# bmhopkinson/hyslam

Measured on AMD Instinct MI355X. Metric: stereo frames/sec ORB extract+match, 1920x1080 @2000 feat, higher is better.
Workload: dtype u8

## Files before the change

### hyslam_amd/csrc/hs_api.hip

```cpp
#include "hs_plan.h"
#include "hs_track.h"
#include <atomic>
#include <climits>
#include <cmath>
#include <cstdio>
#include <cstring>
#include <mutex>
#include <string>
#include <vector>

#define HS_VERSION "hyslam_amd 0.1 (gfx950)"

template <class T, bool Pinned = false> struct HsBuf {
    T* p = nullptr; size_t cap = 0;
    HsBuf() = default;
    HsBuf(const HsBuf&) = delete; HsBuf& operator=(const HsBuf&) = delete;
    HsBuf(HsBuf&& o) noexcept : p(o.p), cap(o.cap) { o.p = nullptr; o.cap = 0; }
    HsBuf& operator=(HsBuf&& o) noexcept { if (this != &o) { release(); p = o.p; cap = o.cap; o.p = nullptr; o.cap = 0; } return *this; }
    ~HsBuf() { release(); }
    void release() { if (p) (void)(Pinned ? hipHostFree(p) : hipFree(p)); p = nullptr; cap = 0; }
    hipError_t grow(size_t count)
    {
        if (count <= cap) return hipSuccess;
        release();
        const hipError_t e = Pinned ? hipHostMalloc((void**)&p, count * sizeof(T), hipHostMallocDefault) : hipMalloc((void**)&p, count * sizeof(T));
        if (e != hipSuccess) { p = nullptr; return e; }
        cap = count;
        return Pinned ? hipSuccess : hs_poison_fresh(p, count * sizeof(T));
    }
    hipError_t grow(size_t count, hipStream_t drain)
    {
        if (count <= cap) return hipSuccess;
        const hipError_t e = hipStreamSynchronize(drain);
        return e != hipSuccess ? e : grow(count);
    }
    operator T*() const { return p; }
};
template <class T> using HsPinned = HsBuf<T, true>;

struct HsFrameStaging { HsBuf<uint8_t> d_in, d_raw; };
struct HsStereoOut {
    HsBuf<float> ur, depth; HsBuf<int32_t> bd;
    hipError_t grow(size_t entries, hipStream_t drain)
    {
        if (entries <= ur.cap && entries <= depth.cap && entries <= bd.cap) return hipSuccess;
        hipError_t e = hipStreamSynchronize(drain);
        if (e == hipSuccess) e = ur.grow(entries);
        if (e == hipSuccess) e = depth.grow(entries);
        if (e == hipSuccess) e = bd.grow(entries);
        return e;
    }
};

struct hs_orb {
    hs_orb_params p;
    int device = 0;
    std::atomic<bool> owned{true};
    std::atomic<int> refs{1};
    hipStream_t stream = nullptr;
    std::string err;
    uint16_t taps[7];
    HsKnobs knobs{};
    HsFastKnobs fast_knobs{};
    uint32_t fast_epoch = 0;
    hipStream_t s_aux = nullptr; hipEvent_t ev_sfork = nullptr, ev_sjoin = nullptr;
    bool fast_taps = false;
    std::vector<float> scale, inv_scale, sigma2, inv_sigma2;
    std::vector<int> quota;
    struct Geometry {
        int w = 0, h = 0, batch_cap = 0;
        uint64_t plan_digest = 0;
        std::vector<HsLevel> lv;
        std::vector<HsLevel> lv_n;
        int last_batch = 0; HsImg0 last_img0{};
        int last_pyr_launches = 0;
        int total_cells = 0, max_wcell = 1, max_hcell = 1;
        int fast_items = 0;
        int fast_items_n = 0;
        uint64_t cand_img_stride = 0;
        int sel_img_stride = 0;
        int max_kp = 0;
        HsBuf<HsFastItem> d_fast_items, d_fast_items_n;
        HsBuf<uint32_t> d_fast_ovf;
        HsBuf<uint8_t> d_pyr;
        HsBuf<int16_t> d_tables;
        HsBuf<uint8_t> d_qt_tabs;
        HsBuf<uint16_t> d_qkeys; HsBuf<HsFastQt> d_fast_qt;
        HsBuf<uint32_t> d_qhist; HsBuf<unsigned long long> d_qbest; uint32_t qhist_stride = 0, qbest_stride = 0;
        HsBuf<uint8_t> d_qt_rects;
        bool keys_dirty = false;
        HsBuf<uint8_t> d_pyr_tabs;
        std::vector<HsPyrFuse> pyr_fuse;
        std::vector<HsPyrChain> pyr_deep;
        std::vector<HsPyrChain> pyr_chain;
        HsBuf<uint2> d_cand; HsBuf<uint32_t> d_pts_xy, d_pts_sk; HsBuf<uint16_t> d_pt_node;
        HsBuf<int32_t> d_cand_count, d_sel_count, d_cell_count;
        HsBuf<uint32_t> d_sel;
        HsBuf<uint16_t> d_sel_perm;
    } geo;
    HsBuf<HsLevel> d_lv;
    HsBuf<uint16_t> d_taps;
    bool qt_large = false;
    bool qt_small_ok = false;
    bool keep_points = false;
    HsFrameStaging in;
    HsBuf<uint8_t> d_out;
    HsStereoOut st;
    HsBuf<int32_t> d_strip_count; HsBuf<HsStripEntry> d_strip_list;
    HsBuf<hs_keypoint> d_sm_kps; HsBuf<uint8_t> d_sm_desc; HsBuf<int32_t> d_sm_n;
    HsPinned<uint8_t> h_pin;
    HsPinned<uint8_t> h_pin_out;
    int last_stereo_launches = 2;
    const hs_keypoint* pub_kps = nullptr; const uint8_t* pub_desc = nullptr; int pub_cap = 0, pub_batch = 0;
    HsBuf<uint8_t> d_scratch;
    struct IngestSlot {
        HsFrameStaging in;
        HsBuf<uint8_t> d_out;
        HsPinned<uint8_t> h_out;
        hipEvent_t ev_in = nullptr, ev_done = nullptr, ev_out = nullptr;
        int32_t ticket = 0; bool busy = false;
        int batch = 0, pairs = 0, cap = 0;
    } slot[2];
    hipStream_t s_in = nullptr, s_out = nullptr;
    int32_t next_ticket = 1;
    hs_orb* lane2 = nullptr; hipEvent_t ev_fork = nullptr, ev_join = nullptr;
    bool prof = false;
    std::vector<hipEvent_t> ev_pool; size_t ev_used = 0;
    std::vector<int> prof_stage;
};

namespace {

inline int cv_round_f(float v) { return (int)nearbyintf(v); }

void mark(hs_orb* h, int stage, hipStream_t s)
{
    if (!h->prof) return;
    if (h->ev_used == h->ev_pool.size()) { hipEvent_t e; if (hipEventCreate(&e) != hipSuccess) return; h->ev_pool.push_back(e); }
    (void)hipEventRecord(h->ev_pool[h->ev_used++], s);
    h->prof_stage.push_back(stage);
}

void free_geometry(hs_orb* h) { h->geo = hs_orb::Geometry{}; }

template <class T> void relocate(T*& p, const void* base) { p = reinterpret_cast<T*>(reinterpret_cast<uintptr_t>(base) + reinterpret_cast<uintptr_t>(p)); }
void relocate_levels(std::vector<HsLevel>& lv, const hs_orb::Geometry& g)
{
    for (size_t l = 0; l < lv.size(); l++) {
        HsLevel& V = lv[l];
        if (l > 0) { relocate(V.base, g.d_pyr.p); relocate(V.xofs, g.d_tables.p); relocate(V.ialpha, g.d_tables.p); relocate(V.yofs, g.d_tables.p); relocate(V.ibeta, g.d_tables.p); }
        if (V.qt_ytab) { relocate(V.qt_xtab, g.d_qt_tabs.p); relocate(V.qt_ytab, g.d_qt_tabs.p); }
    }
}
void relocate_pyramid(hs_orb::Geometry& g)
{
    for (std::vector<HsPyrChain>* plan : { &g.pyr_chain, &g.pyr_deep })
        for (size_t l = 0; l < plan->size(); l++) {
            HsPyrChain& C = (*plan)[l];
            if (!C.valid) continue;
            if (l > 1) relocate(C.sbase, g.d_pyr.p);
            for (int i = 0; i < C.nstage; i++) {
                HsPyrStage& S = C.st[i];
                relocate(S.base, g.d_pyr.p); relocate(S.xt, g.d_tables.p);
                relocate(S.rows, g.d_pyr_tabs.p); relocate(S.tx, g.d_pyr_tabs.p); relocate(S.ty, g.d_pyr_tabs.p);
            }
        }
    for (size_t l = 0; l < g.pyr_fuse.size(); l++) {
        HsPyrFuse& F = g.pyr_fuse[l];
        if (!F.valid) continue;
        if (l > 1) relocate(F.sbase, g.d_pyr.p);
        relocate(F.abase, g.d_pyr.p); relocate(F.bbase, g.d_pyr.p); relocate(F.xtA, g.d_tables.p); relocate(F.xtB, g.d_tables.p);
        relocate(F.rowA, g.d_pyr_tabs.p); relocate(F.rowB, g.d_pyr_tabs.p); relocate(F.xt, g.d_pyr_tabs.p); relocate(F.yt, g.d_pyr_tabs.p);
    }
}
template <class T, class V> hipError_t upload(const HsBuf<T>& d, const std::vector<V>& v)
{
    return v.empty() ? hipSuccess : hipMemcpy(d.p, v.data(), v.size() * sizeof(V), hipMemcpyHostToDevice);
}

int configure_impl(hs_orb* h, int w, int hh, int batch);
int configure(hs_orb* h, int w, int hh, int batch)
{
    if (w == h->geo.w && hh == h->geo.h && batch <= h->geo.batch_cap) return HS_OK;
    if (w < 1 || hh < 1 || w > 16384 || hh > 16384 || batch < 1 || batch > 65535)
        return hs_fail(h, HS_ERR_INVALID, "image size / batch out of range");
    const int rc = configure_impl(h, w, hh, batch);
    if (rc != HS_OK) free_geometry(h);
    return rc;
}
int configure_impl(hs_orb* h, int w, int hh, int batch)
{
    HIP_TRY(h, hipStreamSynchronize(h->stream));
    free_geometry(h);
    hs_orb::Geometry& g = h->geo;
    const int L = h->p.nlevels;
    HsPlan P; std::string refusal;
    const HsPlanInput in{ &h->p, h->inv_scale.data(), h->scale.data(), h->quota.data(), &h->knobs, &h->fast_knobs, h->qt_large, w, hh };
    const int rc = hs_plan_geometry(in, P, refusal);
    if (rc != HS_OK) return hs_fail(h, rc, refusal);
    g.total_cells = P.total_cells; g.max_wcell = P.max_wcell; g.max_hcell = P.max_hcell; g.fast_items = P.fast_items; g.fast_items_n = P.fast_items_n;
    g.cand_img_stride = P.cand_img_stride; g.sel_img_stride = P.sel_img_stride; g.max_kp = P.max_kp;
    g.qhist_stride = P.qhist_stride; g.qbest_stride = P.qbest_stride; g.plan_digest = P.digest;
    g.lv = std::move(P.lv); g.lv_n = std::move(P.lv_n);
    g.pyr_fuse = std::move(P.pyr_fuse); g.pyr_chain = std::move(P.pyr_chain); g.pyr_deep = std::move(P.pyr_deep);

    HIP_TRY(h, g.d_pyr.grow(std::max<size_t>(P.pyr_per_img * batch, 256)));
    HIP_TRY(h, g.d_tables.grow(std::max<size_t>(P.tables.size(), 256 / sizeof(int16_t))));
    const size_t ce = std::max<uint64_t>(g.cand_img_stride * batch, 64);
    HIP_TRY(h, g.d_cand.grow(ce));
    HIP_TRY(h, g.d_pts_xy.grow(ce));
    HIP_TRY(h, g.d_pts_sk.grow(ce));
    HIP_TRY(h, g.d_pt_node.grow(ce));
    if (h->qt_large) HIP_TRY(h, g.d_qt_rects.grow((size_t)batch * L * hs_quadtree_large_scratch_bytes()));
    HIP_TRY(h, g.d_cell_count.grow(std::max<size_t>((size_t)g.total_cells * batch, 64 / 4)));
    HIP_TRY(h, g.d_cand_count.grow((size_t)batch * L));
    HIP_TRY(h, g.d_sel_count.grow((size_t)batch * L));
    HIP_TRY(h, g.d_sel.grow(std::max<size_t>((size_t)g.sel_img_stride * batch * 3, 64 / 4)));
    HIP_TRY(h, g.d_sel_perm.grow(std::max<size_t>((size_t)g.sel_img_stride * batch, 64 / 2)));
    HIP_TRY(h, g.d_qt_tabs.grow(std::max<size_t>(P.qt_tabs.size() + 16, 256)));
    HIP_TRY(h, g.d_qkeys.grow(std::max<size_t>(P.qkeys.size() + 16 / 2, 256 / 2)));
    HIP_TRY(h, g.d_fast_qt.grow(HS_MAX_LEVELS));
    HIP_TRY(h, g.d_qhist.grow(std::max<size_t>((size_t)g.qhist_stride * batch, 256 / 4)));
    HIP_TRY(h, g.d_qbest.grow(std::max<size_t>((size_t)g.qbest_stride * batch, 256 / 8)));
    HIP_TRY(h, g.d_pyr_tabs.grow(std::max<size_t>(P.pyr_tabs.size() * 8, 256)));
    HIP_TRY(h, g.d_fast_items.grow(P.items.size()));
    HIP_TRY(h, g.d_fast_items_n.grow(P.items_n.size()));
    HIP_TRY(h, g.d_fast_ovf.grow(std::max<size_t>(hs_fast_overflow_bytes(g.max_hcell, std::max(g.fast_items, g.fast_items_n) * batch, h->fast_knobs), 256) / 4));

    relocate_levels(g.lv, g); relocate_levels(g.lv_n, g);
    relocate_pyramid(g);
    for (size_t l = 0; l < P.fast_qt.size(); l++) if (P.fast_qt[l].enabled) { relocate(P.fast_qt[l].xkey, g.d_qkeys.p); relocate(P.fast_qt[l].ykey, g.d_qkeys.p); }
    for (std::vector<HsFastItem>* items : { &P.items, &P.items_n })
        for (HsFastItem& it : *items) if (it.level > 0) relocate(it.base, g.d_pyr.p);

    HIP_TRY(h, upload(g.d_tables, P.tables));
    HIP_TRY(h, upload(g.d_qt_tabs, P.qt_tabs));
    HIP_TRY(h, upload(g.d_qkeys, P.qkeys));
    HIP_TRY(h, upload(g.d_fast_qt, P.fast_qt));
    HIP_TRY(h, upload(g.d_pyr_tabs, P.pyr_tabs));
    HIP_TRY(h, hipMemcpy(h->d_lv, g.lv.data(), sizeof(HsLevel) * L, hipMemcpyHostToDevice));
    HIP_TRY(h, hipMemcpy(h->d_lv + L, g.lv_n.data(), sizeof(HsLevel) * L, hipMemcpyHostToDevice));
    HIP_TRY(h, upload(g.d_fast_items, P.items));
    HIP_TRY(h, upload(g.d_fast_items_n, P.items_n));

    HIP_TRY(h, hipMemsetAsync(g.d_qhist, 0, std::max<size_t>((size_t)g.qhist_stride * batch * 4, 256), h->stream));
    HIP_TRY(h, hipMemsetAsync(g.d_qbest, 0, std::max<size_t>((size_t)g.qbest_stride * batch * 8, 256), h->stream));
    HIP_TRY(h, hipMemsetAsync(g.d_fast_ovf, 0, 4 * HS_FAST_QUEUE_DWORDS * 4, h->stream));
    HIP_TRY(h, hipStreamSynchronize(h->stream));
    g.w = w; g.h = hh; g.batch_cap = batch;
    return HS_OK;
}

enum KnobRule { K_ANY, K_FLAG , K_POSITIVE , K_NONNEG , K_MIN2 ,
                K_TRISTATE  };
struct KnobRow { const char* name; int HsKnobs::* field; int def; KnobRule rule; const char* meaning; };
const KnobRow KNOBS[] = {
    { "HS_PYRAMID_NO_FUSE",     &HsKnobs::no_fuse,             0,             K_FLAG,     "one pyramid level per launch (parity tests of the unfused kernel)" },
    { "HS_PYRAMID_CHAIN",       &HsKnobs::chain_mode,          -1,            K_ANY,      "-1 = a three-level chain for the tail of an odd number of levels, 0 = never, 2 = chains for every fused pair too (parity tests)" },
    { "HS_PYRAMID_CHAIN2",      &HsKnobs::pyr_chain2,          0,             K_FLAG,     "HS_PYRAMID_PLAN: a 2 is a two-level chain launch, not the two-level kernel" },
    { "HS_PYRAMID_TBX_MAX",     &HsKnobs::pyr_tbx_max,         0,             K_ANY,      "cap on the level-B tile width of the two-level kernel (experiment: lane utilisation against time)" },
    { "HS_PYRAMID_DEEP_MAX",    &HsKnobs::deep_max_batch,      2,             K_ANY,      "calls of at most this many frames use the small-batch plan (0 = never)" },
    { "HS_PYRAMID_DEEP_ROWS",   &HsKnobs::deep_rows,           8,             K_MIN2,     "rows of the LAST level per tile in the small-batch plan" },
    { "HS_FAST_ORDER",          &HsKnobs::fast_order,          1,             K_ANY,      "order of an image's FAST work items: 1 = reduced levels deepest first, level 0 last; 0 = level 0 first (the order until round 3); 2 = reduced levels interleaved, level 0 last" },
    { "HS_FAST_KEYS",           &HsKnobs::fast_keys,           1,             K_FLAG,     "0: the quadtree kernel gathers the candidates and computes the keys itself (the scheme until round 3)" },
    { "HS_FAST_KEYS_LEVELS",    &HsKnobs::fast_keys_levels,    HS_MAX_LEVELS, K_POSITIVE, "only the levels 0 .. n-1 get keys (tuning)" },
    { "HS_FAST_KEYS_MAX_BATCH", &HsKnobs::fast_keys_max_batch, 16,            K_NONNEG,   "calls of more frames than this run without the keys (see run_extract)" },
    { "HS_QT_POINT_DOMAIN",     &HsKnobs::qt_point_domain,     0,             K_FLAG,     "the quadtree's general point-domain passes only (parity tests of the fallback)" },
    { "HS_QT_SMALL",            &HsKnobs::qt_small,            0,             K_FLAG,     "the quadtree kernel's small instance (two workgroups per CU) where every level's list fits it" },
    { "HS_STEREO_FUSE",         &HsKnobs::stereo_fuse,         1,             K_FLAG,     "0: the stereo front end with a separate k_stereo_strips launch instead of the strips binned by an extra workgroup of the describe launch" },
    { "HS_EXTRACT_SPLIT",       &HsKnobs::split_mode,          -1,            K_TRISTATE, "1 = always run level 0's FAST + quadtree beside the pyramid, 0 = never, unset = for small batches (hs_orb_set_split overrides)" },
};
HsKnobs read_knobs()
{
    HsKnobs k{};
    for (const KnobRow& r : KNOBS) {
        int& dst = k.*r.field;
        dst = r.def;
        const char* e = getenv(r.name);
        if (!e) continue;
        const int v = atoi(e);
        switch (r.rule) {
        case K_ANY: dst = v; break;
        case K_FLAG: dst = v != 0; break;
        case K_POSITIVE: if (v > 0) dst = v; break;
        case K_NONNEG: if (v >= 0) dst = v; break;
        case K_MIN2: if (v >= 2) dst = v; break;
        case K_TRISTATE: dst = v == INT_MIN ? -1 : (v != 0 ? 1 : 0); break;
        }
    }
    if (const char* e = getenv("HS_PYRAMID_PLAN")) { k.pyr_plan_set = true; k.pyr_plan = e; }
    return k;
}

struct OutLayout { size_t off_k, off_d, off_u, off_z, bytes; };
OutLayout out_layout(int batch, int cap, int pairs)
{
    OutLayout o;
    o.off_k = hs_up256((size_t)batch * 4);
    o.off_d = o.off_k + hs_up256((size_t)batch * cap * sizeof(hs_keypoint));
    const size_t desc = (size_t)batch * cap * HS_DESC_BYTES, ur = (size_t)pairs * cap * 4;
    o.off_u = o.off_z = o.bytes = o.off_d + desc;
    if (pairs > 0) { o.off_u = o.off_d + hs_up256(desc); o.off_z = o.off_u + hs_up256(ur); o.bytes = o.off_z + ur; }
    return o;
}

void scatter_results(const uint8_t* blk, const OutLayout& o, int batch, int cap0, int pairs, hs_keypoint* kps, uint8_t* desc, int32_t* n, int cap, float* uRight, float* depth)
{
    memcpy(n, blk, (size_t)batch * 4);
    for (int i = 0; i < batch; i++) {
        const size_t cnt = (size_t)std::min(std::max(n[i], 0), cap0);
        memcpy(kps + (size_t)i * cap, blk + o.off_k + (size_t)i * cap0 * sizeof(hs_keypoint), cnt * sizeof(hs_keypoint));
        memcpy(desc + (size_t)i * cap * HS_DESC_BYTES, blk + o.off_d + (size_t)i * cap0 * HS_DESC_BYTES, cnt * HS_DESC_BYTES);
        if (i < pairs) {
            memcpy(uRight + (size_t)i * cap, blk + o.off_u + (size_t)i * cap0 * 4, cnt * 4);
            memcpy(depth + (size_t)i * cap, blk + o.off_z + (size_t)i * cap0 * 4, cnt * 4);
        }
    }
}

int ensure_stereo_strips(hs_orb* h, int pairs, int cap, int n_rows)
{
    if (n_rows > 65536) return hs_fail(h, HS_ERR_INVALID, "stereo: more than 65536 image rows");
    const size_t need_count = (size_t)pairs * hs_stereo_strips(n_rows);
    HIP_TRY(h, h->d_strip_count.grow(need_count, h->stream));
    HIP_TRY(h, h->d_strip_list.grow(need_count * (size_t)cap, h->stream));
    return HS_OK;
}

int run_extract(hs_orb* h, HsImg0 img0, int batch, HsOut out, hipStream_t s, const HsStripFuse* sf = nullptr)
{
    const int L = h->p.nlevels;
    hs_orb::Geometry& g = h->geo;
    const int narrow_max = h->fast_knobs.narrow_max > 0 ? h->fast_knobs.narrow_max : 18000;
    const bool narrow = g.fast_items_n > 0 && (h->fast_knobs.cols == 32 || (h->fast_knobs.cols != 64 && (long long)g.fast_items_n * batch <= narrow_max));
    const HsPyrChain* const deep = (batch <= h->knobs.deep_max_batch && !g.pyr_deep.empty()) ? g.pyr_deep.data() : nullptr;
    const bool use_keys = h->knobs.fast_keys && g.d_fast_qt.p != nullptr && batch <= h->knobs.fast_keys_max_batch;
    if (g.keys_dirty) {
        HIP_TRY(h, hipDeviceSynchronize());
        if (g.d_qhist) HIP_TRY(h, hipMemsetAsync(g.d_qhist, 0, (size_t)g.qhist_stride * g.batch_cap * 4, s));
        if (g.d_qbest) HIP_TRY(h, hipMemsetAsync(g.d_qbest, 0, (size_t)g.qbest_stride * g.batch_cap * 8, s));
        HIP_TRY(h, hipStreamSynchronize(s));
        g.keys_dirty = false;
    }
    if (use_keys) g.keys_dirty = true;
    const std::vector<HsLevel>& lvh = narrow ? h->geo.lv_n : h->geo.lv;
    const HsLevel* const d_lv = h->d_lv + (narrow ? L : 0);
    const HsFastItem* const d_items = narrow ? g.d_fast_items_n.p : g.d_fast_items.p;
    const int n_items = narrow ? g.fast_items_n : g.fast_items, lc = narrow ? 5 : 6;
    const int items0 = lvh[0].ngroups * lvh[0].nrows, first0 = lvh[0].item_begin;
    const bool split = !h->prof && L > 1 && items0 > 0 && items0 < n_items && (h->knobs.split_mode == 1 || (h->knobs.split_mode < 0 && batch <= 2 && (size_t)g.w * (size_t)g.h * (size_t)batch >= 6000000));
    auto fast = [&](int item_first, int item_count, int spill_slot, hipStream_t st) -> int {
        const bool launched = hs_launch_fast(d_lv, d_items, L, img0, batch, g.total_cells, n_items, h->p.fast_threshold,
                                             g.d_cand, g.d_cell_count, g.cand_img_stride, g.max_wcell, g.max_hcell, g.d_fast_ovf, h->fast_epoch, h->fast_knobs,
                                             item_first, item_count, spill_slot, lc, use_keys ? g.d_fast_qt.p : nullptr, g.d_qhist, g.d_qbest, g.qhist_stride, g.qbest_stride, st);
        const hipError_t e = hipGetLastError();
        if (e != hipSuccess) {
            (void)hipDeviceSynchronize();
            (void)hipMemsetAsync(g.d_fast_ovf, 0, 4 * HS_FAST_QUEUE_DWORDS * 4, h->stream);
            if (g.d_qhist) (void)hipMemsetAsync(g.d_qhist, 0, (size_t)g.qhist_stride * g.batch_cap * 4, h->stream);
            if (g.d_qbest) (void)hipMemsetAsync(g.d_qbest, 0, (size_t)g.qbest_stride * g.batch_cap * 8, h->stream);
            (void)hipStreamSynchronize(h->stream);
            return hs_fail(h, HS_ERR_HIP, std::string("FAST launch: ") + hipGetErrorString(e));
        }
        if (launched) h->fast_epoch++;
        return HS_OK;
    };
    auto quadtree = [&](int level_first, int level_count, hipStream_t st) {
        hs_launch_quadtree(d_lv, L, batch, g.total_cells, g.d_cand, g.d_cell_count, g.cand_img_stride,
                           g.d_pts_xy, g.d_pts_sk, g.d_pt_node, g.d_cand_count, g.d_sel, g.d_sel_count, g.sel_img_stride, g.d_sel_perm, h->knobs.qt_point_domain ? 1 : 0,
                           level_first, level_count, use_keys ? g.d_qhist.p : nullptr, g.d_qbest, g.qhist_stride, g.qbest_stride, h->keep_points ? 1 : 0,
                           h->qt_large ? 2 : (h->qt_small_ok ? 1 : 0), g.d_qt_rects, st);
    };
    if (split) {
        if (!h->s_aux) {
            HIP_TRY(h, hipStreamCreateWithFlags(&h->s_aux, hipStreamNonBlocking));
            HIP_TRY(h, hipEventCreateWithFlags(&h->ev_sfork, hipEventDisableTiming));
            HIP_TRY(h, hipEventCreateWithFlags(&h->ev_sjoin, hipEventDisableTiming));
        }
        HIP_TRY(h, hipEventRecord(h->ev_sfork, s));
        HIP_TRY(h, hipStreamWaitEvent(h->s_aux, h->ev_sfork, 0));
        int rc = fast(first0, items0, 1, h->s_aux);
        if (rc != HS_OK) return rc;
        quadtree(0, 1, h->s_aux);
        HIP_TRY(h, hipEventRecord(h->ev_sjoin, h->s_aux));
        h->geo.last_pyr_launches = hs_launch_pyramid(h->d_lv, h->geo.lv.data(), g.pyr_fuse.data(), g.pyr_chain.data(), L, img0, batch, s, deep);
        rc = fast(0, n_items - items0, 0, s);
        if (rc != HS_OK) return rc;
        quadtree(1, L - 1, s);
        HIP_TRY(h, hipStreamWaitEvent(s, h->ev_sjoin, 0));
    } else {
        mark(h, 0, s);
        h->geo.last_pyr_launches = hs_launch_pyramid(h->d_lv, h->geo.lv.data(), g.pyr_fuse.data(), g.pyr_chain.data(), L, img0, batch, s, deep);
        mark(h, 1, s);
        const int rc = fast(0, n_items, 0, s);
        if (rc != HS_OK) return rc;
        mark(h, 2, s);
        quadtree(0, L, s);
    }
    mark(h, 3, s);
    hs_launch_describe(h->d_lv, L, img0, batch, g.d_sel, g.d_sel_count, g.d_sel_perm, g.sel_img_stride, g.max_kp,
                       h->d_taps, out, s, h->fast_taps, sf ? *sf : HsStripFuse{});
    mark(h, -1, s);
    HIP_TRY(h, hipGetLastError());
    g.keys_dirty = false;
    h->geo.last_batch = batch; h->geo.last_img0 = img0;
    return HS_OK;
}

struct DevFrame { hs_keypoint* kps; uint8_t* desc; int8_t* cell; };
void stage_frame(HsStage& st, const hs_frame_view* F, DevFrame* o)
{
    st.in(&o->kps, F->n, F->kps); st.in(&o->desc, (size_t)F->n * 32, F->desc);
    st.temp(&o->cell, hs_frame_grid_bytes(std::max(F->n, 1)));
}

void run_stereo(hs_orb* h, bool binned, const hs_keypoint* kL, const uint8_t* dL, const int32_t* nL, const hs_keypoint* kR, const uint8_t* dR,
                const int32_t* nR, int pairs, int cap, const hs_stereo_params& sp, float* ur, float* depth, hipStream_t s)
{
    mark(h, 4, s);
    h->last_stereo_launches = binned ? 1 : 2;
    if (binned) hs_launch_stereo_match_only(kL, dL, nL, kR, dR, nR, pairs, cap, sp, ur, depth, h->st.bd, h->d_strip_count, h->d_strip_list, s);
    else hs_launch_stereo(kL, dL, nL, kR, dR, nR, pairs, cap, sp, ur, depth, h->st.bd, h->d_strip_count, h->d_strip_list, s);
    mark(h, 5, s);
    hs_launch_stereo_median(nL, pairs, cap, ur, depth, h->st.bd, sp.th_high, h->d_strip_count, sp.n_rows, s);
    mark(h, -1, s);
}

int run_stereo_frontend(hs_orb* h, HsImg0 img0, HsOut out, const hs_stereo_params& sp, float* ur, float* depth, hipStream_t s)
{
    const int pairs = out.split;
    const HsStripFuse sf{ 1, sp.n_rows, hs_stereo_strips(sp.n_rows), 0, sp.size_ref, h->d_strip_count, h->d_strip_list };
    const int rc = run_extract(h, img0, 2 * pairs, out, s, h->knobs.stereo_fuse ? &sf : nullptr);
    if (rc != HS_OK) return rc;
    run_stereo(h, h->knobs.stereo_fuse, out.kps, out.desc, out.n, out.kps2, out.desc2, out.n2, pairs, out.cap, sp, ur, depth, s);
    HIP_TRY(h, hipGetLastError());
    return HS_OK;
}

template <class Body> int run_lanes(hs_orb* h, hipStream_t s, int count, Body body)
{
    hs_orb* const child = h->lane2;
    const int c0 = count / 2;
    child->prof = h->prof;
    HIP_TRY(h, hipEventRecord(h->ev_fork, s));
    HIP_TRY(h, hipStreamWaitEvent(child->stream, h->ev_fork, 0));
    int rc = body(h, 0, c0, s);
    if (rc == HS_OK) {
        rc = body(child, c0, count - c0, child->stream);
        if (rc != HS_OK) h->err = child->err;
    }
    HIP_TRY(h, hipEventRecord(h->ev_join, child->stream));
    HIP_TRY(h, hipStreamWaitEvent(s, h->ev_join, 0));
    return rc;
}

}

void hs_debug_plan_summary(const hs_orb* h, int32_t* out )
{
    for (int i = 0; i < 8; i++) out[i] = 0;
    if (!h || h->geo.lv.empty()) return;
    const int L = h->p.nlevels;
    out[0] = hs_pyramid_launch_count(h->geo.lv.data(), L);
    int deep_launches = 0, longest = 0, lds = 0;
    for (int l = 1; l < L; l++) {
        deep_launches++;
        if (l < (int)h->geo.pyr_deep.size() && h->geo.pyr_deep[l].valid) {
            const HsPyrChain& C = h->geo.pyr_deep[l];
            if (C.nstage > longest) { longest = C.nstage; lds = C.x_bytes + C.h_rows * 512; }
            l += C.nstage - 1;
        } else if (h->geo.lv[l].chain_n > 0 && l + h->geo.lv[l].chain_n <= L) l += h->geo.lv[l].chain_n - 1;
        else if (h->geo.lv[l].fuse_tbx > 0 && l + 1 < L) l++;
    }
    out[1] = L > 1 ? deep_launches : 0; out[2] = h->geo.fast_items; out[3] = h->geo.fast_items_n;
    for (int l = 0; l < L; l++) out[4] += h->geo.lv[l].qt_hist_off != 0xFFFFFFFFu;
    out[5] = longest; out[6] = lds;
    if (L > 1 && !h->geo.pyr_deep.empty() && h->geo.pyr_deep[1].valid) out[7] = h->geo.pyr_deep[1].grid_x * h->geo.pyr_deep[1].grid_y;
}
uint64_t hs_debug_plan_digest(const hs_orb* h) { return h && h->geo.w > 0 ? h->geo.plan_digest : 0; }

std::atomic<int> g_hs_poison{-1};
static std::atomic<long long> g_hs_poison_violations{0};
void hs_poison_violation() { g_hs_poison_violations.fetch_add(1, std::memory_order_relaxed); }
hipError_t hs_poison_fill(void* p, size_t bytes, int byte)
{
    const hipError_t e = hipMemset(p, byte, bytes);
    return e != hipSuccess ? e : hipStreamSynchronize(nullptr);
}
__global__ __launch_bounds__(256) void k_poison_check(const uint8_t* __restrict__ base, const HsPoisonGaps g, int byte, unsigned long long* __restrict__ first)
{
    const int gap = blockIdx.x;
    if (gap >= g.n) return;
    const unsigned long long e = g.end[gap];
    unsigned long long m = ~0ull;
    for (unsigned long long i = g.begin[gap] + threadIdx.x; i < e; i += 256)
        if (base[i] != (uint8_t)byte) { m = i; break; }
    if (m != ~0ull) atomicMin(first + gap, m);
}
void hs_launch_poison_check(const uint8_t* d_base, const HsPoisonGaps& gaps, int byte, unsigned long long* d_first, hipStream_t s)
{
    if (gaps.n <= 0) return;
    hipLaunchKernelGGL(k_poison_check, dim3(gaps.n), dim3(256), 0, s, d_base, gaps, byte, d_first);
}

void hs_set_error(hs_orb* h, const char* msg) { if (h) h->err = msg ? msg : ""; }
int hs_orb_device_of(const hs_orb* h) { return h ? h->device : 0; }
hipStream_t hs_orb_stream_of(const hs_orb* h) { return h ? h->stream : nullptr; }
uint8_t* hs_orb_scratch_of(hs_orb* h, size_t bytes, hipStream_t user)
{
    const auto claim = [&]() -> int {
        if (bytes > h->d_scratch.cap && user != h->stream) HIP_TRY(h, hipStreamSynchronize(user));
        HIP_TRY(h, h->d_scratch.grow(bytes, h->stream));
        return HS_OK;
    };
    return claim() == HS_OK ? h->d_scratch.p : nullptr;
}

extern "C" {

const char* hs_version(void) { return HS_VERSION; }

const char* hs_status_string(int s)
{
    switch (s) {
    case HS_OK: return "ok";
    case HS_ERR_INVALID: return "invalid argument";
    case HS_ERR_HIP: return "HIP runtime error";
    case HS_ERR_CAPACITY: return "output capacity too small";
    case HS_ERR_NO_DEVICE: return "no usable device";
    case HS_ERR_POISON: return "workspace poison check failed";
    default: return "unknown status";
    }
}

int hs_device_count(int* count)
{
    if (!count) return HS_ERR_INVALID;
    int n = 0;
    if (hipGetDeviceCount(&n) != hipSuccess) { *count = 0; return HS_ERR_NO_DEVICE; }
    *count = n;
    return HS_OK;
}

void hs_orb_default_params(hs_orb_params* p)
{
    if (!p) return;
    memset(p, 0, sizeof(*p));
    p->nfeatures = 1000; p->scale_factor = 1.2f; p->nlevels = 8; p->cell_px = 30;
    p->ini_th_fast = 20; p->min_th_fast = 4;
    p->fast_threshold = 20;
    static const uint16_t t[7] = { 18, 34, 49, 55, 49, 34, 18 };
    memcpy(p->blur_taps, t, sizeof(t));
}

int hs_orb_create(const hs_orb_params* p, int device, hs_orb** out)
{
    if (!p || !out) return HS_ERR_INVALID;
    *out = nullptr;
    if (p->nlevels < 1 || p->nlevels > HS_MAX_LEVELS || p->nfeatures < 1 || !(p->scale_factor > 1.0f) || p->cell_px < 8 ||
        p->fast_threshold < 0 || p->fast_threshold > 255)
        return HS_ERR_INVALID;
    int ndev = 0;
    if (hipGetDeviceCount(&ndev) != hipSuccess || ndev < 1 || device < 0 || device >= ndev) return HS_ERR_NO_DEVICE;
    hs_orb* h = new hs_orb();
    h->p = *p; h->device = device;
    h->fast_knobs = hs_fast_read_knobs();
    h->knobs = read_knobs();
    bool zero = true; for (int k = 0; k < 7; k++) zero = zero && p->blur_taps[k] == 0;
    static const uint16_t def[7] = { 18, 34, 49, 55, 49, 34, 18 };
    for (int k = 0; k < 7; k++) h->taps[k] = zero ? def[k] : p->blur_taps[k];
    { uint32_t sum = 0; bool bytes = true; for (int k = 0; k < 7; k++) { sum += h->taps[k]; bytes = bytes && h->taps[k] <= 255; } h->fast_taps = bytes && sum * 255u <= 0xFFFFu; }

    const int L = p->nlevels;
    const double scaleFactor = p->scale_factor;
    h->scale.resize(L); h->inv_scale.resize(L); h->sigma2.resize(L); h->inv_sigma2.resize(L); h->quota.resize(L);
    h->scale[0] = 1.0f; h->sigma2[0] = 1.0f;
    for (int i = 1; i < L; i++) { h->scale[i] = (float)(h->scale[i - 1] * scaleFactor); h->sigma2[i] = h->scale[i] * h->scale[i]; }
    for (int i = 0; i < L; i++) { h->inv_scale[i] = 1.0f / h->scale[i]; h->inv_sigma2[i] = 1.0f / h->sigma2[i]; }
    float factor = (float)(1.0f / scaleFactor);
    float nDesired = p->nfeatures * (1 - factor) / (1 - (float)pow((double)factor, (double)L));
    int sum = 0;
    for (int l = 0; l < L - 1; l++) { h->quota[l] = cv_round_f(nDesired); sum += h->quota[l]; nDesired *= factor; }
    h->quota[L - 1] = std::max(p->nfeatures - sum, 0);
    for (int l = 0; l < L; l++)
        if (h->quota[l] + 8 > HS_QT_LARGE_NODES) { delete h; return HS_ERR_INVALID; }
    for (int l = 0; l < L; l++) if (h->quota[l] + 8 > HS_QT_MAX_NODES) h->qt_large = true;
    h->qt_small_ok = true;
    for (int l = 0; l < L; l++) if (h->quota[l] + 8 > hs_quadtree_small_nodes()) h->qt_small_ok = false;
    if (!h->knobs.qt_small) h->qt_small_ok = false;

    if (hipSetDevice(device) != hipSuccess) { delete h; return HS_ERR_NO_DEVICE; }
    if (hipStreamCreateWithFlags(&h->stream, hipStreamNonBlocking) != hipSuccess ||
        h->d_lv.grow(2 * HS_MAX_LEVELS) != hipSuccess ||
        h->d_taps.grow(8) != hipSuccess ||
        hipMemcpy(h->d_taps, h->taps, 14, hipMemcpyHostToDevice) != hipSuccess) {
        hs_orb_destroy(h);
        return HS_ERR_HIP;
    }
    *out = h;
    return HS_OK;
}

static void orb_destroy_now(hs_orb* h);
void hs_orb_destroy(hs_orb* h)
{
    if (!h) return;
    h->owned.store(false);
    if (h->refs.fetch_sub(1) == 1) orb_destroy_now(h);
}
int hs_orb_borrowers(const hs_orb* h) { return h ? std::max(0, h->refs.load() - (h->owned.load() ? 1 : 0)) : 0; }
}
void hs_orb_borrow(hs_orb* h, int delta)
{
    if (!h) return;
    if (h->refs.fetch_add(delta) + delta == 0) orb_destroy_now(h);
}
static void orb_destroy_now(hs_orb* h)
{
    hipSetDevice(h->device);
    if (h->lane2) { hs_orb_destroy(h->lane2); h->lane2 = nullptr; }
    if (h->ev_fork) hipEventDestroy(h->ev_fork);
    if (h->ev_join) hipEventDestroy(h->ev_join);
    if (h->s_aux) { hipStreamSynchronize(h->s_aux); hipStreamDestroy(h->s_aux); }
    if (h->ev_sfork) hipEventDestroy(h->ev_sfork);
    if (h->ev_sjoin) hipEventDestroy(h->ev_sjoin);
    if (h->stream) hipStreamSynchronize(h->stream);
    if (h->s_in) hipStreamSynchronize(h->s_in);
    if (h->s_out) hipStreamSynchronize(h->s_out);
    for (auto& sl : h->slot) {
        if (sl.ev_in) hipEventDestroy(sl.ev_in);
        if (sl.ev_done) hipEventDestroy(sl.ev_done);
        if (sl.ev_out) hipEventDestroy(sl.ev_out);
    }
    if (h->s_in) hipStreamDestroy(h->s_in);
    if (h->s_out) hipStreamDestroy(h->s_out);
    for (hipEvent_t e : h->ev_pool) hipEventDestroy(e);
    if (h->stream) hipStreamDestroy(h->stream);
    delete h;
}
extern "C" {

const char* hs_orb_last_error(const hs_orb* h) { return h ? h->err.c_str() : "null handle"; }
int hs_orb_get_levels(const hs_orb* h) { return h ? h->p.nlevels : 0; }
int hs_orb_get_device(const hs_orb* h) { return h ? h->device : -1; }
float hs_orb_get_scale_factor(const hs_orb* h) { return h ? (float)(double)h->p.scale_factor : 0.f; }

int hs_orb_get_scale_tables(const hs_orb* h, float* scale, float* inv_scale, float* sigma2, float* inv_sigma2, int32_t* fpl)
{
    if (!h) return HS_ERR_INVALID;
    for (int i = 0; i < h->p.nlevels; i++) {
        if (scale) scale[i] = h->scale[i];
        if (inv_scale) inv_scale[i] = h->inv_scale[i];
        if (sigma2) sigma2[i] = h->sigma2[i];
        if (inv_sigma2) inv_sigma2[i] = h->inv_sigma2[i];
        if (fpl) fpl[i] = h->quota[i];
    }
    return HS_OK;
}

int hs_orb_max_keypoints(const hs_orb* h)
{
    if (!h) return 0;
    int n = 0;
    for (int l = 0; l < h->p.nlevels; l++) n += std::max(h->quota[l] + 4, 4 * 8 + 4);
    return std::max(n, h->geo.max_kp);
}

int hs_orb_reserve(hs_orb* h, int w, int h_px, int batch)
{
    if (!h) return HS_ERR_INVALID;
    HIP_TRY(h, hipSetDevice(h->device));
    return configure(h, w, h_px, batch);
}

int hs_orb_extract_batch_device(hs_orb* h, const uint8_t* d_imgs, int batch, int w, int h_px,
                                size_t row_stride, size_t image_stride,
                                hs_keypoint* d_kps, uint8_t* d_desc, int32_t* d_n, int cap, void* stream)
{
    if (!h) return HS_ERR_INVALID;
    if (!d_imgs || !d_kps || !d_desc || !d_n || batch < 1 || row_stride < (size_t)w || cap < 1 || cap > 65535)
        return hs_fail(h, HS_ERR_INVALID, "bad argument");
    if (((uintptr_t)d_desc & 15) != 0 || (((uintptr_t)d_kps | (uintptr_t)d_n) & 3) != 0)
        return hs_fail(h, HS_ERR_INVALID, "output alignment: descriptors 16 bytes (they are written with 16-byte vector stores; hs_record_offsets pads for it), keypoints and counts 4");
    HIP_TRY(h, hipSetDevice(h->device));
    hipStream_t s = hs_stream_or(h, stream);
    const auto body = [&](hs_orb* q, int first, int count, hipStream_t qs) -> int {
        int rc = configure(q, w, h_px, count);
        if (rc != HS_OK) return rc;
        if (cap < q->geo.max_kp) return hs_fail(q, HS_ERR_CAPACITY, "cap < keypoints this frame size can produce; see hs_orb_max_keypoints");
        const uint8_t* const imgs = d_imgs + (size_t)first * image_stride;
        hs_keypoint* const k = d_kps + (size_t)first * cap; uint8_t* const d = d_desc + (size_t)first * cap * HS_DESC_BYTES;
        HsImg0 img0{ imgs, imgs, count, (uint64_t)row_stride, (uint64_t)image_stride };
        HsOut out{ k, d, d_n + first, k, d, d_n + first, count, cap };
        return run_extract(q, img0, count, out, qs);
    };
    return h->lane2 && batch >= 2 ? run_lanes(h, s, batch, body) : body(h, 0, batch, s);
}

namespace {
struct FramePlan {
    int w, h, gw, gh;
    size_t pitch, per_img;
    size_t row_bytes, rpitch, raw_img;
};
int plan_frames(hs_orb* h, int w, int h_px, const hs_preprocess_params* pp, FramePlan* u)
{
    u->w = u->gw = w; u->h = u->gh = h_px;
    if (pp) hs_preprocess_out_size(w, h_px, pp->scale, &u->gw, &u->gh);
    if (u->gw < 1 || u->gh < 1) return hs_fail(h, HS_ERR_INVALID, "the camera scale reduces the frame to nothing (cv::resize asserts on an empty size)");
    u->pitch = ((size_t)u->gw + 63) & ~(size_t)63; u->per_img = u->pitch * u->gh;
    u->row_bytes = (size_t)w * (pp ? pp->channels : 1);
    u->rpitch = pp ? (u->row_bytes + 3) & ~(size_t)3 : 0; u->raw_img = u->rpitch * h_px;
    return HS_OK;
}

int upload_frames(hs_orb* h, HsFrameStaging& st, const hipStream_t* drain, const FramePlan& u, bool camera, const uint8_t* const* imgs, int batch, size_t stride, bool linear, hipStream_t s)
{
    HIP_TRY(h, drain ? st.d_in.grow(u.per_img * batch, *drain) : st.d_in.grow(u.per_img * batch));
    if (camera) HIP_TRY(h, drain ? st.d_raw.grow(u.raw_img * batch, *drain) : st.d_raw.grow(u.raw_img * batch));
    uint8_t* const dst = camera ? st.d_raw.p : st.d_in.p;
    const size_t dp = camera ? u.rpitch : u.pitch, di = camera ? u.raw_img : u.per_img;
    for (int i = 0; i < batch; i++) {
        if (linear && stride == dp && u.row_bytes == dp) HIP_TRY(h, hipMemcpyAsync(dst + di * i, imgs[i], di, hipMemcpyHostToDevice, s));
        else HIP_TRY(h, hipMemcpy2DAsync(dst + di * i, dp, imgs[i], stride, u.row_bytes, u.h, hipMemcpyHostToDevice, s));
    }
    return HS_OK;
}

int preprocess_frames(hs_orb* h, const HsFrameStaging& st, const FramePlan& u, const hs_preprocess_params& pp, int batch, hipStream_t s)
{
    hs_launch_preprocess(st.d_raw, u.w, u.h, u.rpitch, u.raw_img, pp.channels, pp.rgb, pp.scale, st.d_in, u.gw, u.gh, u.pitch, u.per_img, 1, batch, s);
    HIP_TRY(h, hipGetLastError());
    return HS_OK;
}

int extract_host_frames(hs_orb* h, const uint8_t* const* imgs, int batch, int w, int h_px, size_t stride, const hs_preprocess_params* pp,
                        hs_keypoint* kps, uint8_t* desc, int cap, int32_t* n, uint8_t* grey_out)
{
    HIP_TRY(h, hipSetDevice(h->device));
    h->pub_kps = nullptr; h->pub_desc = nullptr; h->pub_batch = 0;
    FramePlan u;
    int rc = plan_frames(h, w, h_px, pp, &u);
    if (rc == HS_OK) rc = configure(h, u.gw, u.gh, batch);
    if (rc != HS_OK) return rc;
    if (cap < h->geo.max_kp) return hs_fail(h, HS_ERR_CAPACITY, "cap < keypoints this frame size can produce; see hs_orb_max_keypoints");
    hipStream_t s = h->stream;
    const OutLayout o = out_layout(batch, cap, 0);
    HIP_TRY(h, h->d_out.grow(o.bytes, s));
    for (int i = 0; i < batch; i++) if (!imgs[i]) return hs_fail(h, HS_ERR_INVALID, "null image in batch");
    rc = upload_frames(h, h->in, &s, u, pp != nullptr, imgs, batch, stride, true, s);
    if (rc == HS_OK && pp) rc = preprocess_frames(h, h->in, u, *pp, batch, s);
    if (rc != HS_OK) return rc;
    int32_t* const d_n = reinterpret_cast<int32_t*>(h->d_out.p);
    hs_keypoint* const d_kps = reinterpret_cast<hs_keypoint*>(h->d_out + o.off_k); uint8_t* const d_desc = h->d_out + o.off_d;
    HsImg0 img0{ h->in.d_in, h->in.d_in, batch, (uint64_t)u.pitch, (uint64_t)u.per_img };
    HsOut out{ d_kps, d_desc, d_n, d_kps, d_desc, d_n, batch, cap };
    rc = run_extract(h, img0, batch, out, s);
    if (rc != HS_OK) return rc;
    HIP_TRY(h, h->h_pin_out.grow(o.bytes, s));
    HIP_TRY(h, hipMemcpyAsync(h->h_pin_out, h->d_out, o.bytes, hipMemcpyDeviceToHost, s));
    if (grey_out) HIP_TRY(h, hipMemcpy2DAsync(grey_out, (size_t)u.gw, h->in.d_in, u.pitch, (size_t)u.gw, (size_t)u.gh * batch, hipMemcpyDeviceToHost, s));
    HIP_TRY(h, hipStreamSynchronize(s));
    scatter_results(h->h_pin_out, o, batch, cap, 0, kps, desc, n, cap, nullptr, nullptr);
    h->pub_kps = d_kps; h->pub_desc = d_desc; h->pub_cap = cap; h->pub_batch = batch;
    return HS_OK;
}
}

int hs_orb_extract_batch(hs_orb* h, const uint8_t* const* imgs, int batch, int w, int h_px, int stride,
                         hs_keypoint* kps, uint8_t* desc, int cap, int32_t* n)
{
    if (!h) return HS_ERR_INVALID;
    if (!n || batch < 1) return hs_fail(h, HS_ERR_INVALID, "bad argument");
    if (w == 0 || h_px == 0 || !imgs) { for (int i = 0; i < batch; i++) n[i] = 0; return HS_OK; }
    if (!kps || !desc || stride < w || cap < 1 || cap > 65535) return hs_fail(h, HS_ERR_INVALID, "bad argument");
    return extract_host_frames(h, imgs, batch, w, h_px, (size_t)stride, nullptr, kps, desc, cap, n, nullptr);
}

void hs_preprocess_size(int w, int h_px, float scale, int32_t* ow, int32_t* oh)
{
// ... 990 lines not shown
```

### hyslam_amd/csrc/hs_internal.h

```cpp
#pragma once
#include <algorithm>
#include <atomic>
#include <string>
#include <type_traits>
#include <vector>
#include <hip/hip_runtime.h>
#include <stdint.h>
#include <stddef.h>
#include "../../include/hyslam_amd.h"
#include "hs_work.h"

#define HS_MAX_LEVELS 16
#define HS_EDGE 19
#define HS_BORDER 16
#define HS_MAX_CELL_H 125
#define HS_QT_MAX_NODES 2048
#define HS_QT_LARGE_NODES 3328
#define HS_QT_THREADS 1024

struct HsLevel {
    int32_t w, h;
    int32_t pitch;
    int32_t _r0;
    uint64_t img_stride;
    uint8_t* base;
    int32_t ncols, nrows, wcell, hcell;
    int32_t cell_begin;
    int32_t grp_cells, ngroups;
    int32_t item_begin;
    int32_t inv_wcell, inv_wcell1;
    int32_t qt_w, qt_h;
    int32_t n_ini;
    float   hx;
    int32_t quota;
    const uint8_t* qt_xtab;
    const uint8_t* qt_ytab;
    int32_t qt_rbound[8];
    uint32_t qt_hist_off;
    uint32_t qt_best_off;
    int32_t cand_cap;
    int32_t sel_cap;
    uint64_t cand_off;
    int32_t sel_off;
    int32_t xmax;
    const int16_t* xofs;
    const int16_t* ialpha;
    const int16_t* yofs;
    const int16_t* ibeta;
    float scale;
    float kp_size;
    int32_t fuse_tbx, fuse_ar, fuse_sr, fuse_pitch;
    int32_t chain_n;
    int32_t _r1;
};

struct HsFastItem {
    const uint8_t* base;
    uint64_t img_stride;
    int32_t pitch;
    int32_t gcell0;
    int32_t c0;
    uint32_t slot0;
    int32_t ccap;
    int32_t inv_w, inv_w1;
    uint16_t iniY, a0;
    uint16_t th, iw;
    uint8_t off, ndw, ncell, level;
    uint16_t xoff, yoff;
    uint32_t _pad;
};
static_assert(sizeof(HsFastItem) == 64, "HsFastItem is fetched as one 64-byte record");

struct HsFastQt { const uint16_t* xkey; const uint16_t* ykey; uint32_t hist_off, best_off; int32_t enabled, _r; };
static_assert(sizeof(HsFastQt) == 32, "scalar-load record");

__host__ __device__ inline int hs_cell_cap(int wcell, int hcell) { return ((((wcell + 1) >> 1) * ((hcell + 1) >> 1)) + 3) & ~3; }

struct HsImg0 {
    const uint8_t* base;
    const uint8_t* base2;
    int32_t split;
    uint64_t row_stride;
    uint64_t img_stride;
};
__host__ __device__ inline const uint8_t* hs_img0_ptr(const HsImg0& I, int img)
{
    return img < I.split ? I.base + (size_t)img * I.img_stride : I.base2 + (size_t)(img - I.split) * I.img_stride;
}

#define HS_GLOBAL __attribute__((address_space(1)))
typedef uint32_t hs_u32x4 __attribute__((ext_vector_type(4)));
template <typename T> __device__ __forceinline__ T hs_gload(const void* p) { return *(const HS_GLOBAL T*)(uintptr_t)p; }
#define HS_CONSTANT __attribute__((address_space(4)))
template <typename T> __device__ __forceinline__ T hs_cload(const void* p) { return *(const HS_CONSTANT T*)(uintptr_t)p; }
__device__ __forceinline__ int hs_cload_i16(const int16_t* base, int idx)
{
    const uint32_t w = hs_cload<uint32_t>(reinterpret_cast<const uint8_t*>(base) + 4 * (size_t)(idx >> 1));
    return (int)(int16_t)((idx & 1) ? (w >> 16) : (w & 0xFFFFu));
}
__device__ __forceinline__ const uint8_t* hs_uniform_ptr(const uint8_t* p)
{
    const uint64_t v = (uint64_t)(uintptr_t)p;
    const uint32_t lo = __builtin_amdgcn_readfirstlane((uint32_t)v), hi = __builtin_amdgcn_readfirstlane((uint32_t)(v >> 32));
    return (const uint8_t*)(uintptr_t)(((uint64_t)hi << 32) | lo);
}
template <typename T> __device__ __forceinline__ T hs_gload_off(const uint8_t* uniform_base, uint32_t lane_off)
{
    return *(const HS_GLOBAL T*)((const HS_GLOBAL uint8_t*)(uintptr_t)uniform_base + lane_off);
}
template <typename T> __device__ __forceinline__ void hs_gstore(void* p, T v) { *(HS_GLOBAL T*)(uintptr_t)p = v; }

struct HsOut {
    hs_keypoint* kps; uint8_t* desc; int32_t* n;
    hs_keypoint* kps2; uint8_t* desc2; int32_t* n2;
    int32_t split;
    int32_t cap;
};

struct HsXTab { int16_t sx, a0, a1, pad; };
struct HsPyrXTile { int32_t ax0, own_x1, col0, nvec, _r[4]; };
struct HsPyrYTile { int32_t ay0, own_y1, ay_last, sy_first, n_sr, _r[3]; };
struct HsPyrRow { uint16_t off0, off1, b0, b1; };
static_assert(sizeof(HsPyrXTile) == 32 && sizeof(HsPyrYTile) == 32 && sizeof(HsPyrRow) == 8, "scalar-load records");
struct HsPyrFuse {
    const uint8_t* sbase;
    uint64_t s_img_stride; int32_t spitch; int32_t _r0;
    uint8_t* abase; uint64_t a_img_stride; int32_t apitch, aw, ah, slotA;
    uint8_t* bbase; uint64_t b_img_stride; int32_t bpitch, bw, bh, _r2;
    const HsXTab* xtA; const HsXTab* xtB;
    const HsPyrRow* rowA; const HsPyrRow* rowB;
    const HsPyrXTile* xt; const HsPyrYTile* yt;
    int32_t tbx, sr, lds_pitch, valid;
};

struct HsPyrStageX { int32_t x0, own_x1, ncols, src_x0, nvec, _r[3]; };
struct HsPyrStageY { int32_t y0, own_y1, y_last, src_y0, n_src, _r[3]; };
static_assert(sizeof(HsPyrStageX) == 32 && sizeof(HsPyrStageY) == 32, "scalar-load records");
struct HsPyrStage {
    uint8_t* base; uint64_t img_stride; int32_t pitch, w, h, slot;
    const HsXTab* xt; const HsPyrRow* rows;
    const HsPyrStageX* tx; const HsPyrStageY* ty;
};
#define HS_PYR_DEEP_LDS (120 * 1024)
#define HS_PYR_CHAIN_MAX 7
struct HsPyrChain {
    const uint8_t* sbase; uint64_t s_img_stride; int32_t spitch, nstage;
    HsPyrStage st[HS_PYR_CHAIN_MAX];
    int32_t tbx, lds_pitch, x_bytes, h_rows;
    int32_t grid_x, grid_y, valid, _r;
};

#define HS_STRIP_ENTRY_BYTES 16
#define HS_STRIP_SHIFT 5
struct __attribute__((aligned(16))) HsStripEntry { float uR; int32_t octave; uint32_t idx_band; uint32_t _pad; };
static_assert(sizeof(HsStripEntry) == HS_STRIP_ENTRY_BYTES, "hs_api.hip sizes the strip lists with HS_STRIP_ENTRY_BYTES");
#define HS_STRIPS_MAX 2048
struct HsStripFuse { int32_t enabled, n_rows, n_strips, _r; float size_ref; int32_t* strip_count; HsStripEntry* strip_list; };
inline int hs_stereo_strips(int n_rows) { return (n_rows > 0 ? ((n_rows - 1) >> 5) : 0) + 1; }

int  hs_launch_pyramid(const HsLevel* d_lv, const HsLevel* h_lv, const HsPyrFuse* fuse , const HsPyrChain* chain , int nlevels, HsImg0 img0, int batch, hipStream_t s,
                       const HsPyrChain* deep = nullptr );
void hs_pyramid_plan_chain(const HsLevel* h_lv, int first, int n, const int16_t* const* xtab, const int16_t* const* yofs, const int16_t* const* ibeta,
                           std::vector<uint64_t>& blob, HsPyrChain& C, size_t lds_max = 60 * 1024, int tile_rows = 0 );
void hs_pyramid_build_tables(const HsLevel* h_lv, int nlevels, const int16_t* const* xtab, const int16_t* const* yofs, const int16_t* const* ibeta,
                             std::vector<uint64_t>& blob, std::vector<HsPyrFuse>& fuse);
void hs_pyramid_plan_fusion(HsLevel* h_lv, int nlevels, const int16_t* const* xtab , const int16_t* const* yofs , int tbx_max = 0 );
int hs_pyramid_launch_count(const HsLevel* h_lv, int nlevels);
int hs_fast_group_cells(int wcell, int ncols, int lc);
int hs_fast_max_cell_w(int lc);
void hs_fast_build_items(const HsLevel* h_lv, int nlevels, HsFastItem* out );
bool hs_fast_item_fits(const HsFastItem& it, int lc);
#define HS_FAST_NQ_MAX 32
#define HS_FAST_QUEUE_DWORDS (32 * HS_FAST_NQ_MAX)
struct HsFastKnobs { int pcap, small_lists, wg_per_cu, force_scan_b, image_major, nq, cols, narrow_max, no_fold, list_min; };
HsFastKnobs hs_fast_read_knobs();
bool hs_launch_fast(const HsLevel* d_lv, const HsFastItem* d_items, int nlevels, HsImg0 img0, int batch, int total_cells, int items_per_img, int fast_th,
                    uint2* cand , int32_t* cell_count, uint64_t cand_img_stride,
                    int max_wcell, int max_hcell, uint32_t* overflow , uint32_t epoch ,
                    const HsFastKnobs& knobs, int item_first, int item_count ,
                    int spill_slot , int lc ,
                    const HsFastQt* d_qt , uint32_t* qhist, unsigned long long* qbest, uint32_t qhist_img_stride, uint32_t qbest_img_stride, hipStream_t s);
size_t hs_fast_overflow_bytes(int max_hcell, int total_work_max, const HsFastKnobs& knobs);
bool hs_quadtree_build_tables(HsLevel& V, std::vector<uint8_t>& blob, size_t& xoff, size_t& yoff);
void hs_launch_quadtree(const HsLevel* d_lv, int nlevels, int batch, int total_cells,
                        const uint2* cand, const int32_t* cell_count, uint64_t cand_img_stride,
                        uint32_t* pts_xy, uint32_t* pts_sk, uint16_t* pt_node, int32_t* cand_count,
                        uint32_t* sel_xys, int32_t* sel_count, int sel_img_stride, uint16_t* sel_perm , int force_point_domain, int level_first, int level_count,
                        uint32_t* qhist , unsigned long long* qbest, uint32_t qhist_img_stride, uint32_t qbest_img_stride,
                        int keep_points ,
                        int list_mode ,
                        uint8_t* rect_scratch , hipStream_t s);
void hs_preprocess_out_size(int w, int h, float fscale, int* ow, int* oh);
int  hs_preprocess_mode(int w, int h, int ow, int oh, float fscale);
void hs_launch_preprocess(const uint8_t* d_src, int sw, int sh, size_t src_row_stride, size_t src_img_stride, int channels, int rgb, float fscale,
                          uint8_t* d_dst, int dw, int dh, size_t dst_row_stride, size_t dst_img_stride, int dst_may_pad ,
                          int batch, hipStream_t s);
int hs_quadtree_small_nodes();
size_t hs_quadtree_large_scratch_bytes();
void hs_launch_describe(const HsLevel* d_lv, int nlevels, HsImg0 img0, int batch,
                        const uint32_t* sel_xys, const int32_t* sel_count, const uint16_t* sel_perm, int sel_img_stride, int max_sel,
                        const uint16_t* taps7, HsOut out, hipStream_t s, bool fast_taps, HsStripFuse strips);
void hs_launch_stereo(const hs_keypoint* kpsL, const uint8_t* descL, const int32_t* nL,
                      const hs_keypoint* kpsR, const uint8_t* descR, const int32_t* nR,
                      int pairs, int cap, hs_stereo_params sp, float* uRight, float* depth,
                      int32_t* best_dist ,
                      int32_t* strip_count , void* strip_list , hipStream_t s);
void hs_launch_stereo_median(const int32_t* nL, int pairs, int cap, float* uRight, float* depth, const int32_t* best_dist, float th_high,
                             int32_t* strip_count , int n_rows, hipStream_t s);
void hs_launch_stereo_match_only(const hs_keypoint* kpsL, const uint8_t* descL, const int32_t* nL,
                                 const hs_keypoint* kpsR, const uint8_t* descR, const int32_t* nR,
                                 int pairs, int cap, hs_stereo_params sp, float* uRight, float* depth, int32_t* best_dist,
                                 const int32_t* strip_count, const void* strip_list, hipStream_t s);

size_t hs_frame_grid_bytes(int n);
void hs_launch_frame_grid(const hs_frame_view& F, const hs_keypoint* d_kps, int8_t* d_cell , bool with_lists, hipStream_t s);
void hs_launch_search_projection(const hs_frame_view& F, const hs_keypoint* d_kps, const uint8_t* d_desc, const float* d_uR,
                                 const int32_t* d_obs, const int8_t* d_cell, const hs_landmark* d_lms, int L, const hs_proj_params& pp,
                                 int32_t* d_match_idx, float* d_match_dist, int32_t* d_winner, float* d_prev_angle_scratch,
                                 int32_t* d_n_matches, hipStream_t s, const hs_pose_view* d_pose = nullptr );
void hs_launch_bow(const int32_t* d_pair_a, const int32_t* d_pair_b, int n_pairs,
                   const int32_t* d_ptr1, const int32_t* d_idx1, const int32_t* d_ptr2, const int32_t* d_idx2,
                   const uint8_t* d_desc1, const uint8_t* d_desc2, const uint8_t* d_keep1, const uint8_t* d_keep2,
                   const float* F12, float size_ref, float sigma_ref, float thr, float ratio,
                   int32_t* d_match12, int n1, const hs_keypoint* d_kps1, const hs_keypoint* d_kps2, float* d_angle2_scratch,
                   int check_rotation, int32_t* d_self_scratch, int32_t* d_n_matches, hipStream_t s);
void hs_launch_knn2(const uint8_t* d_q, int nq, const uint8_t* d_t, int nt, int32_t* d_bi, int32_t* d_bd, int32_t* d_sd, hipStream_t s);
void hs_launch_sim3_projection(const hs_frame_view& F, const hs_keypoint* d_kps, const uint8_t* d_desc, const int8_t* d_cell,
                               const float* R9, const float* t3, const float* Ow3, const hs_landmark* d_lms, int L, float th, float th_low,
                               float* d_geo, uint8_t* d_kp_matched, int32_t* d_match_idx, int32_t* d_n_matches, hipStream_t s);
void hs_launch_sim3_search(const hs_frame_view& F1, const hs_keypoint* d_kps1, const uint8_t* d_desc1, const int8_t* d_cell1,
                           const hs_frame_view& F2, const hs_keypoint* d_kps2, const uint8_t* d_desc2, const int8_t* d_cell2,
                           const hs_landmark* d_lms1, const hs_landmark* d_lms2, const float* sR21, const float* t21, const float* sR12, const float* t12,
                           float th, float th_high, int32_t* d_m1, int32_t* d_m2, int32_t* d_match12, int32_t* d_n_found, hipStream_t s);
void hs_launch_knn2_records(const uint8_t* d_recs, size_t stride, int world, int rank, int cap, size_t off_desc,
                            int32_t* d_bi, int32_t* d_bd, int32_t* d_sd, hipStream_t s);
void hs_launch_stream_copy(void* d_dst, const void* d_src, size_t bytes, int width, hipStream_t s);
void hs_launch_bow_legacy(const int32_t* d_pair_a, const int32_t* d_pair_b, int n_pairs,
                          const int32_t* d_ptr1, const int32_t* d_idx1, const int32_t* d_ptr2, const int32_t* d_idx2,
                          const uint8_t* d_desc1, const uint8_t* d_desc2, const uint8_t* d_keep1, const uint8_t* d_keep2, float thr, float ratio,
                          int32_t* d_match12, int n1, int n2, const hs_keypoint* d_kps1, const hs_keypoint* d_kps2, float* d_angle1_scratch,
                          int check_orientation, int32_t* d_self_scratch, uint32_t* d_taken2, int32_t* d_n_matches, hipStream_t s);
void hs_launch_bow_transform(int n, const uint8_t* d_desc, const int32_t* d_cb, const int32_t* d_cc, const uint8_t* d_ndesc, const int32_t* d_word,
                             const float* d_weight, int levels, int levelsup, int32_t* d_out_word, float* d_out_weight, int32_t* d_out_node, hipStream_t s);
void hs_launch_search_init(const hs_frame_view& F2, const hs_keypoint* d_kps2, const uint8_t* d_desc2, const int8_t* d_cell2,
                           const hs_keypoint* d_kps1, const uint8_t* d_desc1, int n1, const float* d_prev_xy, float window, float th_low, float nnratio,
                           int32_t* d_owner, int32_t* d_odist, float* d_angle_scratch, int32_t* d_self_scratch, int32_t* d_n_matches, hipStream_t s);

void hs_launch_local_keyframes(int n_kf, const int32_t* d_weights, const uint8_t* d_kf_bad, const int32_t* d_neigh, int neigh_cap, const int32_t* d_parent,
                               int n_max, int n_neighbor, uint8_t* d_local, int32_t* d_n_local, hipStream_t s);
void hs_launch_local_points(const hs_kf_table& T, const uint8_t* d_local, const int32_t* d_frame_lm, int n_assoc, uint8_t* d_frame_remove,
                            int32_t* d_sel, int cap, int32_t* d_n_sel, const HsLocalPointsWork& w, hipStream_t s);
void hs_launch_landmark_gather(const hs_landmark* d_lms, int L, const int32_t* d_sel, const int32_t* d_n_sel, int cap, hs_landmark* d_out, hipStream_t s);
void hs_launch_local_map_query(int n_assoc, int64_t* d_q_off, hipStream_t s);

void hs_set_error(hs_orb* h, const char* msg);
int hs_orb_device_of(const hs_orb* h);
hipStream_t hs_orb_stream_of(const hs_orb* h);
uint8_t* hs_orb_scratch_of(hs_orb* h, size_t bytes, hipStream_t user);
inline hipStream_t hs_stream_or(const hs_orb* h, void* stream) { return stream ? (hipStream_t)stream : hs_orb_stream_of(h); }

inline int hs_fail(hs_orb* h, int code, const std::string& msg) { hs_set_error(h, msg.c_str()); return code; }
#define HIP_TRY(h, expr) do { hipError_t e__ = (expr); if (e__ != hipSuccess) { (void)hipGetLastError(); \
    return hs_fail(h, HS_ERR_HIP, std::string(#expr) + ": " + hipGetErrorString(e__)); } } while (0)

inline const char* hs_bad(bool refused) { return refused ? "bad argument" : nullptr; }
template <class Enqueue> int hs_device_call(hs_orb* h, const char* why, void* stream, Enqueue enqueue)
{
    if (!h) return HS_ERR_INVALID;
    if (why) return hs_fail(h, HS_ERR_INVALID, why);
    HIP_TRY(h, hipSetDevice(hs_orb_device_of(h)));
    if constexpr (std::is_void<decltype(enqueue(hipStream_t()))>::value) enqueue(hs_stream_or(h, stream));
    else { const int rc = enqueue(hs_stream_or(h, stream)); if (rc != HS_OK) return rc; }
    HIP_TRY(h, hipGetLastError());
    return HS_OK;
}

inline bool hs_csr_ok(const int64_t* off, int n)
{
    if (off[0] < 0) return false;
    for (int i = 0; i < n; i++) if (off[i + 1] < off[i]) return false;
    return true;
}
inline bool hs_index_range_ok(const int32_t* v, size_t n, int lo, int limit)
{
    for (size_t i = 0; i < n; i++) if (v[i] < lo || v[i] >= limit) return false;
    return true;
}

#define HS_STAGE_MAX_PIECES 17
#define HS_STAGE_SLACK 4096

extern std::atomic<int> g_hs_poison;
inline int hs_poison_byte() { return g_hs_poison.load(std::memory_order_relaxed); }
hipError_t hs_poison_fill(void* p, size_t bytes, int byte);
inline hipError_t hs_poison_fresh(void* p, size_t bytes) { const int b = hs_poison_byte(); return b < 0 || !p || !bytes ? hipSuccess : hs_poison_fill(p, bytes, b); }
struct HsPoisonGaps { int32_t n, _r; unsigned long long begin[HS_STAGE_MAX_PIECES], end[HS_STAGE_MAX_PIECES]; };
#define HS_POISON_REPORT_BYTES 256
void hs_launch_poison_check(const uint8_t* d_base, const HsPoisonGaps& gaps, int byte, unsigned long long* d_first, hipStream_t s);
void hs_poison_violation();

class HsStage {
public:
    explicit HsStage(hs_orb* h) : h_(h), s_(hs_orb_stream_of(h)) {}
    HsStage(hs_orb* h, hipStream_t s) : h_(h), s_(s) {}
    hipStream_t stream() const { return s_; }
    template <class T> void temp(T** d, size_t count) { add(d, count * sizeof(T), nullptr, nullptr, 0); }
    template <class T> void in(T** d, size_t count, const T* src) { add(d, count * sizeof(T), src, nullptr, 0); }
    template <class T> void out(T** d, size_t count, T* dst, size_t n_back = SIZE_MAX) { add(d, count * sizeof(T), nullptr, dst, std::min(n_back, count) * sizeof(T)); }
    template <class T> void inout(T** d, size_t count, T* host) { add(d, count * sizeof(T), host, host, count * sizeof(T)); }
    int begin()
    {
        if (n_ > HS_STAGE_MAX_PIECES) return hs_fail(h_, HS_ERR_INVALID, "internal: a host call stages more than HS_STAGE_MAX_PIECES pieces");
        poison_ = hs_poison_byte();
        const size_t claim = total_ + HS_STAGE_SLACK;
        uint8_t* base = hs_orb_scratch_of(h_, claim + (poison_ >= 0 ? HS_POISON_REPORT_BYTES : 0), s_);
        if (!base) return HS_ERR_HIP;
        if (poison_ >= 0) {
            base_ = base;
            HIP_TRY(h_, hipMemsetAsync(base, poison_, claim, s_));
            HIP_TRY(h_, hipMemsetAsync(base + claim, 0xFF, HS_POISON_REPORT_BYTES, s_));
        }
        for (int i = 0; i < n_; i++) {
            const Piece& p = p_[i];
            *p.dev = base + p.off;
            if (p.src && p.bytes) HIP_TRY(h_, hipMemcpyAsync(*p.dev, p.src, p.bytes, hipMemcpyHostToDevice, s_));
        }
        return HS_OK;
    }
    int finish()
    {
        HIP_TRY(h_, hipGetLastError());
        unsigned long long first[HS_STAGE_MAX_PIECES];
        if (poison_ >= 0) { const int rc = check_enqueue(first); if (rc != HS_OK) return rc; }
        for (int i = 0; i < n_; i++)
            if (p_[i].back) HIP_TRY(h_, hipMemcpyAsync(p_[i].dst, *p_[i].dev, p_[i].back, hipMemcpyDeviceToHost, s_));
        HIP_TRY(h_, hipStreamSynchronize(s_));
        return poison_ >= 0 ? check_report(first) : HS_OK;
    }
    int verify()
    {
        if (poison_ < 0) return HS_OK;
        unsigned long long first[HS_STAGE_MAX_PIECES];
        const int rc = check_enqueue(first);
        if (rc != HS_OK) return rc;
        HIP_TRY(h_, hipStreamSynchronize(s_));
        return check_report(first);
    }
private:
    struct Piece { void** dev; size_t off, bytes, back; const void* src; void* dst; };
    template <class T> void add(T** d, size_t bytes, const void* src, void* dst, size_t back)
    {
        if (n_ < HS_STAGE_MAX_PIECES) { p_[n_] = Piece{ reinterpret_cast<void**>(d), total_, bytes, back, src, dst }; total_ += hs_up256(std::max<size_t>(bytes, 1)); }
        n_++;
    }
    int check_enqueue(unsigned long long* first)
    {
        if (n_ == 0) return HS_OK;
        HsPoisonGaps g{};
        g.n = n_;
        for (int i = 0; i < n_; i++) { g.begin[i] = p_[i].off + p_[i].bytes; g.end[i] = i + 1 < n_ ? p_[i + 1].off : total_ + HS_STAGE_SLACK; }
        unsigned long long* d_first = reinterpret_cast<unsigned long long*>(base_ + total_ + HS_STAGE_SLACK);
        hs_launch_poison_check(base_, g, poison_, d_first, s_);
        HIP_TRY(h_, hipGetLastError());
        HIP_TRY(h_, hipMemcpyAsync(first, d_first, (size_t)n_ * sizeof(unsigned long long), hipMemcpyDeviceToHost, s_));
        return HS_OK;
    }
    int check_report(const unsigned long long* first)
    {
        for (int i = 0; i < n_; i++) {
            if (first[i] == ~0ull) continue;
            hs_poison_violation();
            const bool slack = i + 1 == n_ && first[i] >= total_;
            return hs_fail(h_, HS_ERR_POISON, "workspace poison: piece " + std::to_string(i) + " (arena offset " + std::to_string(p_[i].off) + ", " + std::to_string(p_[i].bytes) +
                           " bytes) was written past its end: first changed byte at arena offset " + std::to_string(first[i]) + (slack ? " (in the slack)" : " (in its padding)"));
        }
        return HS_OK;
    }
    hs_orb* h_; hipStream_t s_; int n_ = 0; size_t total_ = 0; Piece p_[HS_STAGE_MAX_PIECES];
    int poison_ = -1; uint8_t* base_ = nullptr;
};
```

### hyslam_amd/csrc/hs_plan.h

```cpp
#pragma once
#include "hs_internal.h"

struct HsKnobs {
    int no_fuse, stereo_fuse, fast_keys, fast_keys_levels, fast_keys_max_batch, fast_order;
    int chain_mode, pyr_chain2, pyr_tbx_max, deep_max_batch, deep_rows;
    int qt_point_domain, qt_small, split_mode;
    bool pyr_plan_set = false;
    std::string pyr_plan;
};

struct HsPlanInput {
    const hs_orb_params* p;
    const float* inv_scale; const float* scale; const int* quota;
    const HsKnobs* knobs; const HsFastKnobs* fast_knobs;
    bool qt_large;
    int w, h;
};

struct HsPlan {
    int w = 0, h = 0;
    int total_cells = 0, max_wcell = 1, max_hcell = 1, fast_items = 0, fast_items_n = 0;
    uint64_t cand_img_stride = 0; int sel_img_stride = 0, max_kp = 0;
    uint32_t qhist_stride = 0, qbest_stride = 0;
    size_t pyr_per_img = 0;
    std::vector<HsLevel> lv, lv_n;
    std::vector<int16_t> tables;
    std::vector<uint8_t> qt_tabs;
    std::vector<uint16_t> qkeys;
    std::vector<HsFastQt> fast_qt;
    std::vector<uint64_t> pyr_tabs;
    std::vector<HsPyrFuse> pyr_fuse;
    std::vector<HsPyrChain> pyr_chain;
    std::vector<HsPyrChain> pyr_deep;
    std::vector<HsFastItem> items, items_n;
    uint64_t digest = 0;
};

int hs_plan_geometry(const HsPlanInput& in, HsPlan& out, std::string& err);
uint64_t hs_plan_digest(const HsPlan& P);
```

### hyslam_amd/csrc/hs_plan.hip

```cpp
#include "hs_plan.h"
#include <cmath>
#include <cstdlib>
#include <cstring>
#include <type_traits>
#include <utility>

namespace {

inline int cv_round_f(float v) { return (int)nearbyintf(v); }
inline int cv_floor_f(float v) { int i = (int)v; return i - (i > v); }
inline short sat_short(float v) { int i = cv_round_f(v); return (short)(i < -32768 ? -32768 : (i > 32767 ? 32767 : i)); }

template <class T> T* at_offset(size_t bytes) { return reinterpret_cast<T*>((uintptr_t)bytes); }

struct Refusal { int code; const char* text; };
const Refusal OK{ HS_OK, "" };

Refusal plan_levels(const HsPlanInput& in, HsPlan& P)
{
    const int L = in.p->nlevels;
    P.lv.assign(L, HsLevel{});
    size_t pyr_per_img = 0; uint64_t cand = 0; int sel = 0, cells = 0, items = 0;
    for (int l = 0; l < L; l++) {
        HsLevel& V = P.lv[l];
        V.w = cv_round_f((float)in.w * in.inv_scale[l]);
        V.h = cv_round_f((float)in.h * in.inv_scale[l]);
        if (V.w < 1 || V.h < 1) return { HS_ERR_INVALID, "pyramid level collapses to zero size" };
        V.pitch = (V.w + 63) & ~63;
        if (l > 0) { V.base = at_offset<uint8_t>(pyr_per_img); pyr_per_img += (size_t)V.pitch * V.h; }
        const int minB = HS_BORDER, maxBX = V.w - HS_BORDER, maxBY = V.h - HS_BORDER;
        const float width = (float)(maxBX - minB), height = (float)(maxBY - minB);
        const float W = (float)in.p->cell_px;
        V.ncols = width > 0 ? (int)(width / W) : 0;
        V.nrows = height > 0 ? (int)(height / W) : 0;
        if (V.ncols < 1 || V.nrows < 1) { V.ncols = V.nrows = 0; V.wcell = V.hcell = 0; }
        else { V.wcell = (int)ceilf(width / V.ncols); V.hcell = (int)ceilf(height / V.nrows); }
        if (V.wcell > hs_fast_max_cell_w(6) || V.hcell > HS_MAX_CELL_H)
            return { HS_ERR_INVALID, "FAST cell wider than 247 px or taller than 125 px is not supported" };
        V.cell_begin = cells; cells += V.ncols * V.nrows;
        V.grp_cells = hs_fast_group_cells(V.wcell, V.ncols, 6);
        V.ngroups = V.grp_cells > 0 ? (V.ncols + V.grp_cells - 1) / V.grp_cells : 0;
        V.item_begin = items; items += V.ngroups * V.nrows;
        V.inv_wcell = V.wcell > 0 ? (65536 + V.wcell - 1) / V.wcell : 0;
        V.inv_wcell1 = V.wcell > 0 ? (65536 + V.wcell) / (V.wcell + 1) : 0;
        V.qt_w = maxBX - minB; V.qt_h = maxBY - minB;
        V.n_ini = (V.qt_w > 0 && V.qt_h > 0) ? (int)roundf((float)V.qt_w / (float)V.qt_h) : 0;
        if (V.ncols > 0 && V.n_ini < 1) return { HS_ERR_INVALID, "aspect ratio w/h < 0.5 is undefined behaviour in the reference (nIni == 0)" };
        if (V.ncols < 1) V.n_ini = 0;
        if (V.n_ini > (in.qt_large ? HS_QT_LARGE_NODES : HS_QT_MAX_NODES) / 4) return { HS_ERR_INVALID, "aspect ratio too wide" };
        V.hx = V.n_ini > 0 ? (float)V.qt_w / V.n_ini : 1.f;
        V.quota = in.quota[l];
        V.cand_cap = V.ncols * V.nrows * hs_cell_cap(V.wcell, V.hcell);
        V.cand_off = cand; cand += (uint64_t)((V.cand_cap + 3) & ~3);
        V.sel_cap = std::max(V.quota + 4, 4 * V.n_ini + 4);
        V.sel_off = sel; sel += V.sel_cap;
        V.scale = in.scale[l];
        V.kp_size = (float)(int)(31 * in.scale[l]);
    }
    P.pyr_per_img = hs_up256(pyr_per_img);
    for (int l = 0; l < L; l++) {
        P.lv[l].img_stride = P.pyr_per_img;
        P.max_wcell = std::max(P.max_wcell, P.lv[l].wcell); P.max_hcell = std::max(P.max_hcell, P.lv[l].hcell);
    }
    P.w = in.w; P.h = in.h;
    P.total_cells = cells; P.fast_items = items; P.cand_img_stride = cand; P.sel_img_stride = sel; P.max_kp = sel;
    return OK;
}

void plan_resize_tables(HsPlan& P)
{
    std::vector<int16_t>& tables = P.tables;
    for (size_t l = 1; l < P.lv.size(); l++) {
        HsLevel& V = P.lv[l];
        const int sw = P.lv[l - 1].w, sh = P.lv[l - 1].h;
        const double scale_x = 1. / ((double)V.w / sw), scale_y = 1. / ((double)V.h / sh);
        int xmax = V.w;
        auto grow = [&](size_t n) { size_t o = (tables.size() + 3) & ~(size_t)3; tables.resize(o + n); return o; };
        const size_t o0 = grow(4 * (size_t)V.w);
        const size_t o2 = grow(V.h);
        const size_t o3 = grow(2 * (size_t)V.h);
        for (int dx = 0; dx < V.w; dx++) {
            float fx = (float)((dx + 0.5) * scale_x - 0.5);
            int sx = cv_floor_f(fx); fx -= sx;
            if (sx < 0) { fx = 0; sx = 0; }
            if (sx + 1 >= sw) { xmax = std::min(xmax, dx); if (sx >= sw - 1) { fx = 0; sx = sw - 1; } }
            tables[o0 + 4 * dx] = (int16_t)sx;
            tables[o0 + 4 * dx + 1] = sat_short((1.f - fx) * 2048);
            tables[o0 + 4 * dx + 2] = sat_short(fx * 2048);
            tables[o0 + 4 * dx + 3] = 0;
        }
        for (int dy = 0; dy < V.h; dy++) {
            float fy = (float)((dy + 0.5) * scale_y - 0.5);
            int sy = cv_floor_f(fy); fy -= sy;
            tables[o2 + dy] = (int16_t)std::max(-32768, std::min(32767, sy));
            tables[o3 + 2 * dy] = sat_short((1.f - fy) * 2048);
            tables[o3 + 2 * dy + 1] = sat_short(fy * 2048);
        }
        V.xmax = xmax;
        V.xofs = at_offset<int16_t>(2 * o0); V.ialpha = at_offset<int16_t>(2 * o0);
        V.yofs = at_offset<int16_t>(2 * o2); V.ibeta = at_offset<int16_t>(2 * o3);
    }
}

int order_items(std::vector<HsLevel>& lv, int fast_order)
{
    const int L = (int)lv.size();
    int pos = 0;
    if (fast_order == 0) { for (int l = 0; l < L; l++) { lv[l].item_begin = pos; pos += lv[l].ngroups * lv[l].nrows; } }
    else {
        for (int l = L - 1; l >= 1; l--) { lv[l].item_begin = pos; pos += lv[l].ngroups * lv[l].nrows; }
        lv[0].item_begin = pos; pos += lv[0].ngroups * lv[0].nrows;
    }
    return pos;
}

void plan_quadtree_keys(const HsKnobs& k, HsPlan& P)
{
    const int L = (int)P.lv.size();
    std::vector<uint8_t>& qblob = P.qt_tabs;
    std::vector<size_t> xo(L, 0), yo2(L, 0); std::vector<char> has(L, 0);
    for (int l = 0; l < L; l++) {
        has[l] = hs_quadtree_build_tables(P.lv[l], qblob, xo[l], yo2[l]) ? 1 : 0;
        if (has[l]) { P.lv[l].qt_xtab = at_offset<uint8_t>(xo[l]); P.lv[l].qt_ytab = at_offset<uint8_t>(yo2[l]); }
    }
    auto spread = [](uint32_t v) { v = (v | (v << 4)) & 0x0F0Fu; v = (v | (v << 2)) & 0x3333u; v = (v | (v << 1)) & 0x5555u; return v; };
    std::vector<uint16_t>& keys = P.qkeys;
    P.fast_qt.assign(L, HsFastQt{});
    uint32_t hoff = 0, boff = 0;
    for (int l = 0; l < L; l++) {
        HsLevel& V = P.lv[l];
        V.qt_hist_off = V.qt_best_off = 0xFFFFFFFFu;
        if (!has[l] || !k.fast_keys || l >= k.fast_keys_levels) continue;
        const int DH = V.n_ini <= 2 ? 6 : 5, ncell = V.n_ini << (2 * DH);
        const size_t kx = keys.size(); keys.resize(kx + (size_t)V.qt_w + 1 + 512, 0);
        for (int x = 0; x <= V.qt_w; x++) {
            int r = 0;
            for (int i = 1; i < V.n_ini; i++) r += x >= V.qt_rbound[i];
            keys[kx + x] = (uint16_t)(((uint32_t)r << (2 * DH)) | spread(qblob[xo[l] + x]));
        }
        const size_t ky = keys.size(); keys.resize(ky + (size_t)V.qt_h + 1 + 512, 0);
        for (int y = 0; y <= V.qt_h; y++) keys[ky + y] = (uint16_t)(spread(qblob[yo2[l] + y]) << 1);
        V.qt_hist_off = hoff; V.qt_best_off = boff;
        hoff += (uint32_t)(ncell / 2); boff += (uint32_t)ncell;
        HsFastQt& Q = P.fast_qt[l];
        Q.xkey = at_offset<uint16_t>(2 * kx); Q.ykey = at_offset<uint16_t>(2 * ky);
        Q.hist_off = V.qt_hist_off; Q.best_off = V.qt_best_off; Q.enabled = 1;
    }
    P.qhist_stride = hoff; P.qbest_stride = boff;
}

void plan_pyramid(const HsKnobs& k, HsPlan& P)
{
    const int L = (int)P.lv.size();
    std::vector<HsLevel>& lv = P.lv;
    std::vector<const int16_t*> xt(L, nullptr), yo(L, nullptr), ib(L, nullptr);
    for (int l = 1; l < L; l++) {
        const uint8_t* const t = reinterpret_cast<const uint8_t*>(P.tables.data());
        xt[l] = reinterpret_cast<const int16_t*>(t + (uintptr_t)lv[l].xofs); yo[l] = reinterpret_cast<const int16_t*>(t + (uintptr_t)lv[l].yofs);
        ib[l] = reinterpret_cast<const int16_t*>(t + (uintptr_t)lv[l].ibeta);
    }
    hs_pyramid_plan_fusion(lv.data(), L, xt.data(), yo.data(), k.pyr_tbx_max);
    if (k.no_fuse) for (int l = 0; l < L; l++) lv[l].fuse_tbx = 0;
    std::vector<uint64_t>& blob = P.pyr_tabs;
    hs_pyramid_build_tables(lv.data(), L, xt.data(), yo.data(), ib.data(), blob, P.pyr_fuse);
    P.pyr_chain.assign(L, HsPyrChain{});
    for (int l = 0; l < L; l++) lv[l].chain_n = 0;
    if (!k.no_fuse && k.chain_mode != 0) {
        if (k.chain_mode == 2) {
            for (int l = 1; l + 1 < L; l += 2) {
                int n = (l + 3 == L) ? 3 : 2;
                hs_pyramid_plan_chain(lv.data(), l, n, xt.data(), yo.data(), ib.data(), blob, P.pyr_chain[l]);
                if (!P.pyr_chain[l].valid && n == 3) hs_pyramid_plan_chain(lv.data(), l, 2, xt.data(), yo.data(), ib.data(), blob, P.pyr_chain[l]);
                if (P.pyr_chain[l].valid) { lv[l].chain_n = P.pyr_chain[l].nstage; if (P.pyr_chain[l].nstage == 3) l++; }
            }
        } else if (k.pyr_plan_set) {
            const bool chain2 = k.pyr_chain2 != 0;
            int l = 1;
            for (const char* q = k.pyr_plan.c_str(); *q && l < L; ) {
                const int n = std::min(atoi(q), L - l);
                if (n >= 3 || (n == 2 && (chain2 || !(l & 1)))) {
                    hs_pyramid_plan_chain(lv.data(), l, n, xt.data(), yo.data(), ib.data(), blob, P.pyr_chain[l], HS_PYR_DEEP_LDS, 0);
                    if (P.pyr_chain[l].valid) lv[l].chain_n = n;
                }
                if (n == 1) lv[l].fuse_tbx = 0;
                l += std::max(n, 1);
                while (*q && *q != ',') q++;
                if (*q == ',') q++;
            }
        } else if (L >= 4 && ((L - 1) & 1)) {
            const int l = L - 3;
            hs_pyramid_plan_chain(lv.data(), l, 3, xt.data(), yo.data(), ib.data(), blob, P.pyr_chain[l]);
            if (P.pyr_chain[l].valid) lv[l].chain_n = 3;
        }
    }
    P.pyr_deep.assign(L, HsPyrChain{});
    if (!k.no_fuse && k.deep_max_batch > 0) {
        for (int l = 1; l + 1 < L;) {
            int took = 0;
            for (int n = std::min(HS_PYR_CHAIN_MAX, L - l); n >= 2 && !took; n--) {
                hs_pyramid_plan_chain(lv.data(), l, n, xt.data(), yo.data(), ib.data(), blob, P.pyr_deep[l], HS_PYR_DEEP_LDS, k.deep_rows);
                if (P.pyr_deep[l].valid) took = n;
            }
            l += took ? took : 1;
        }
    }
}

Refusal plan_fast_items(const HsKnobs& k, const HsFastKnobs& fk, HsPlan& P)
{
    const int L = (int)P.lv.size();
    P.lv_n = P.lv;
    bool narrow_ok = fk.cols != 64;
    for (int l = 0; l < L; l++) if (P.lv[l].wcell > hs_fast_max_cell_w(5)) narrow_ok = false;
    if (narrow_ok) {
        for (int l = 0; l < L; l++) {
            HsLevel& V = P.lv_n[l];
            V.grp_cells = hs_fast_group_cells(V.wcell, V.ncols, 5);
            V.ngroups = V.grp_cells > 0 ? (V.ncols + V.grp_cells - 1) / V.grp_cells : 0;
        }
        P.fast_items_n = order_items(P.lv_n, k.fast_order);
    }
    bool items_fit = true;
    auto build = [&](const std::vector<HsLevel>& lv, int n_items, std::vector<HsFastItem>& fi, int lc) {
        fi.assign(std::max(n_items, 1), HsFastItem{});
        hs_fast_build_items(lv.data(), L, fi.data());
        for (int i = 0; i < n_items; i++) items_fit = items_fit && hs_fast_item_fits(fi[i], lc);
        if (k.fast_order == 2 && L > 2) {
            const int n_red = lv[0].item_begin;
            std::vector<std::pair<double, int>> key(n_red);
            for (int l = 1; l < L; l++) {
                const int n = lv[l].ngroups * lv[l].nrows;
                for (int j = 0; j < n; j++) key[lv[l].item_begin + j] = { (j + 0.5) / n, lv[l].item_begin + j };
            }
            std::stable_sort(key.begin(), key.end(), [](const std::pair<double, int>& a, const std::pair<double, int>& b) { return a.first < b.first; });
            std::vector<HsFastItem> t(fi.begin(), fi.begin() + n_red);
            for (int i = 0; i < n_red; i++) fi[i] = t[key[i].second];
        }
    };
    build(P.lv, P.fast_items, P.items, 6);
    if (P.fast_items_n > 0) build(P.lv_n, P.fast_items_n, P.items_n, 5);
    if (!items_fit) return { HS_ERR_INVALID, "internal: a FAST work item does not fit its tile (hs_fast_group_cells); geometry refused" };
    return OK;
}

struct Fnv {
    uint64_t v = 0xcbf29ce484222325ull;
    void bytes(const void* p, size_t n)
    {
        const uint8_t* b = static_cast<const uint8_t*>(p);
        for (; n >= 8; n -= 8, b += 8) { uint64_t w; memcpy(&w, b, 8); v ^= w; v *= 0x100000001b3ull; }
        for (; n > 0; n--, b++) { v ^= *b; v *= 0x100000001b3ull; }
    }
    template <class T> void val(const T& x) { static_assert(std::is_arithmetic<T>::value, "fields only: a record may have padding"); bytes(&x, sizeof(T)); }
    void off(const void* p) { val((uint64_t)(uintptr_t)p); }
    template <class T> void vec(const std::vector<T>& x) { val((uint64_t)x.size()); if (!x.empty()) bytes(x.data(), x.size() * sizeof(T)); }
};

void hash_level(Fnv& H, const HsLevel& V)
{
    H.val(V.w); H.val(V.h); H.val(V.pitch); H.val(V._r0); H.val(V.img_stride); H.off(V.base);
    H.val(V.ncols); H.val(V.nrows); H.val(V.wcell); H.val(V.hcell); H.val(V.cell_begin);
    H.val(V.grp_cells); H.val(V.ngroups); H.val(V.item_begin); H.val(V.inv_wcell); H.val(V.inv_wcell1);
    H.val(V.qt_w); H.val(V.qt_h); H.val(V.n_ini); H.val(V.hx); H.val(V.quota);
    H.off(V.qt_xtab); H.off(V.qt_ytab); for (int i = 0; i < 8; i++) H.val(V.qt_rbound[i]);
    H.val(V.qt_hist_off); H.val(V.qt_best_off); H.val(V.cand_cap); H.val(V.sel_cap); H.val(V.cand_off); H.val(V.sel_off);
    H.val(V.xmax); H.off(V.xofs); H.off(V.ialpha); H.off(V.yofs); H.off(V.ibeta); H.val(V.scale); H.val(V.kp_size);
    H.val(V.fuse_tbx); H.val(V.fuse_ar); H.val(V.fuse_sr); H.val(V.fuse_pitch); H.val(V.chain_n); H.val(V._r1);
}

static_assert(sizeof(HsFastQt) == 32 && sizeof(HsPyrFuse) == 152 && sizeof(HsPyrStage) == 64 && sizeof(HsPyrChain) == 56 + 64 * HS_PYR_CHAIN_MAX && sizeof(HsFastItem) == 64,
              "hs_plan_digest hashes these records as bytes: a record that gains padding must be hashed field by field");

}

int hs_plan_geometry(const HsPlanInput& in, HsPlan& P, std::string& err)
{
    P = HsPlan{};
    Refusal r = plan_levels(in, P);
    if (r.code == HS_OK) {
        plan_resize_tables(P);
        order_items(P.lv, in.knobs->fast_order);
        plan_quadtree_keys(*in.knobs, P);
        plan_pyramid(*in.knobs, P);
        r = plan_fast_items(*in.knobs, *in.fast_knobs, P);
    }
    if (r.code != HS_OK) { err = r.text; return r.code; }
    P.digest = hs_plan_digest(P);
    return HS_OK;
}

uint64_t hs_plan_digest(const HsPlan& P)
{
    Fnv H;
    H.val(P.w); H.val(P.h); H.val(P.total_cells); H.val(P.max_wcell); H.val(P.max_hcell); H.val(P.fast_items); H.val(P.fast_items_n);
    H.val(P.cand_img_stride); H.val(P.sel_img_stride); H.val(P.max_kp); H.val(P.qhist_stride); H.val(P.qbest_stride); H.val((uint64_t)P.pyr_per_img);
    for (const std::vector<HsLevel>* lv : { &P.lv, &P.lv_n }) { H.val((uint64_t)lv->size()); for (const HsLevel& V : *lv) hash_level(H, V); }
    H.vec(P.tables); H.vec(P.qt_tabs); H.vec(P.qkeys); H.vec(P.fast_qt); H.vec(P.pyr_tabs);
    H.vec(P.pyr_fuse); H.vec(P.pyr_chain); H.vec(P.pyr_deep);
    H.vec(P.items); H.vec(P.items_n);
    return H.v;
}
```

### hyslam_amd/csrc/kernels_pyramid.hip

```cpp
#include "hs_internal.h"
#include <atomic>
#include <algorithm>
#include <cstring>
#include <cstdlib>

template <bool ALIGNED>
__global__ __launch_bounds__(256) void k_resize_level(const HsLevel* __restrict__ lv, int level, HsImg0 img0)
{
    const HsLevel& D = lv[level];
    const int img = blockIdx.z;
    const int dy = blockIdx.y * 4 + threadIdx.y;
    const int dx0 = (blockIdx.x * 64 + threadIdx.x) * 4;
    if (dy >= D.h || dx0 >= D.w) return;

    const uint8_t* sbase; size_t spitch;
    if (level == 1) { sbase = hs_img0_ptr(img0, img); spitch = img0.row_stride; }
    else { const HsLevel& S = lv[level - 1]; sbase = S.base + (size_t)img * S.img_stride; spitch = S.pitch; }
    const int sw = lv[level - 1].w, sh = lv[level - 1].h;

    const int sy = D.yofs[dy];
    const int b0 = D.ibeta[2 * dy], b1 = D.ibeta[2 * dy + 1];
    const int sy0 = sy < 0 ? 0 : (sy >= sh ? sh - 1 : sy);
    const int sy1 = sy + 1 < 0 ? 0 : (sy + 1 >= sh ? sh - 1 : sy + 1);
    const uint8_t* S0 = sbase + (size_t)sy0 * spitch;
    const uint8_t* S1 = sbase + (size_t)sy1 * spitch;

    const HsXTab* xt = reinterpret_cast<const HsXTab*>(D.xofs);
    HsXTab t[4];
#pragma unroll
    for (int i = 0; i < 4; i++) t[i] = xt[min(dx0 + i, D.w - 1)];

    uint32_t packed = 0;
    const int base = t[0].sx & ~3;
    const int last = min(t[3].sx + 1, sw - 1);
    if (ALIGNED && last - base < 12) {
        uint32_t r0[4], r1[4];
        const uint32_t* p0 = reinterpret_cast<const uint32_t*>(S0 + base);
        const uint32_t* p1 = reinterpret_cast<const uint32_t*>(S1 + base);
#pragma unroll
        for (int j = 0; j < 4; j++) {
            bool need = base + 4 * j <= last;
            r0[j] = need ? p0[j] : 0u;
            r1[j] = need ? p1[j] : 0u;
        }
#pragma unroll
        for (int i = 0; i < 4; i++) {
            const int k = t[i].sx - base;
            const int q = k >> 2;
            uint32_t lo0 = q == 0 ? r0[0] : (q == 1 ? r0[1] : r0[2]), hi0 = q == 0 ? r0[1] : (q == 1 ? r0[2] : r0[3]);
            uint32_t lo1 = q == 0 ? r1[0] : (q == 1 ? r1[1] : r1[2]), hi1 = q == 0 ? r1[1] : (q == 1 ? r1[2] : r1[3]);
            uint32_t w0 = __builtin_amdgcn_alignbyte(hi0, lo0, k & 3);
            uint32_t w1 = __builtin_amdgcn_alignbyte(hi1, lo1, k & 3);
            int s00 = w0 & 0xFF, s01 = (w0 >> 8) & 0xFF, s10 = w1 & 0xFF, s11 = (w1 >> 8) & 0xFF;
            int h0, h1;
            if (dx0 + i < D.xmax) { h0 = s00 * t[i].a0 + s01 * t[i].a1; h1 = s10 * t[i].a0 + s11 * t[i].a1; }
            else { h0 = s00 * 2048; h1 = s10 * 2048; }
            int v = (((b0 * (h0 >> 4)) >> 16) + ((b1 * (h1 >> 4)) >> 16) + 2) >> 2;
            packed |= (uint32_t)(v & 0xFF) << (8 * i);
        }
    } else {
#pragma unroll
        for (int i = 0; i < 4; i++) {
            const int sx = t[i].sx;
            const int sx1 = sx + 1 < sw ? sx + 1 : sw - 1;
            int h0, h1;
            if (dx0 + i < D.xmax) { h0 = S0[sx] * t[i].a0 + S0[sx1] * t[i].a1; h1 = S1[sx] * t[i].a0 + S1[sx1] * t[i].a1; }
            else { h0 = S0[sx] * 2048; h1 = S1[sx] * 2048; }
            int v = (((b0 * (h0 >> 4)) >> 16) + ((b1 * (h1 >> 4)) >> 16) + 2) >> 2;
            packed |= (uint32_t)(v & 0xFF) << (8 * i);
        }
    }
    uint8_t* drow = D.base + (size_t)img * D.img_stride + (size_t)dy * D.pitch;
    *reinterpret_cast<uint32_t*>(drow + dx0) = packed;
}

typedef unsigned short hs_us2 __attribute__((ext_vector_type(2)));
__device__ __forceinline__ uint32_t pyr_hpair(uint32_t whi, uint32_t wlo, uint32_t sel0, uint32_t sel1, uint32_t coef0, uint32_t coef1)
{
    const uint32_t h0 = __builtin_amdgcn_udot2(__builtin_bit_cast(hs_us2, __builtin_amdgcn_perm(whi, wlo, sel0)), __builtin_bit_cast(hs_us2, coef0), 0u, false);
    const uint32_t h1 = __builtin_amdgcn_udot2(__builtin_bit_cast(hs_us2, __builtin_amdgcn_perm(whi, wlo, sel1)), __builtin_bit_cast(hs_us2, coef1), 0u, false);
    return __builtin_amdgcn_perm(h1, h0, 0x06050201u);
}
__device__ __forceinline__ uint32_t pyr_vpix4(uint32_t h0, uint32_t h1, uint32_t b0, uint32_t b1)
{
    const uint32_t p0 = __umul24(h0, b0), p1 = __umul24(h1, b1);
    const uint32_t hi = __builtin_amdgcn_perm(p1, p0, 0x07060302u);
    return __builtin_amdgcn_udot2(__builtin_bit_cast(hs_us2, hi), __builtin_bit_cast(hs_us2, 0x00010001u), 2u, false);
}
__device__ __forceinline__ uint32_t pyr_vquad(uint2 H0, uint2 H1, uint32_t b0, uint32_t b1)
{
    const uint32_t v0 = pyr_vpix4(H0.x & 0xFFFFu, H1.x & 0xFFFFu, b0, b1), v1 = pyr_vpix4(H0.x >> 16, H1.x >> 16, b0, b1);
    const uint32_t v2 = pyr_vpix4(H0.y & 0xFFFFu, H1.y & 0xFFFFu, b0, b1), v3 = pyr_vpix4(H0.y >> 16, H1.y >> 16, b0, b1);
    uint32_t a = v0 | (v1 << 16), c = v2 | (v3 << 16), a2, c2;
    const uint32_t two = 0x00020002u;
    asm("v_pk_lshrrev_b16 %0, %2, %1" : "=v"(a2) : "v"(a), "v"(two));
    asm("v_pk_lshrrev_b16 %0, %2, %1" : "=v"(c2) : "v"(c), "v"(two));
    return __builtin_amdgcn_perm(c2, a2, 0x06040200u);
}

template <int NW>
__device__ __forceinline__ void pyr_stage_source(const uint8_t* src0 , uint32_t spitch, uint8_t* s_dst, uint32_t dpitch, int nvec, int nrows, int tx, int wave)
{
    const int rpw = nvec <= 16 ? 4 : (nvec <= 21 ? 3 : (nvec <= 32 ? 2 : 1));
    const int rl = (tx >= nvec) + (tx >= 2 * nvec) + (tx >= 3 * nvec), q = tx - rl * nvec;
    if (tx >= rpw * nvec) return;
#ifdef HS_PYR_NOLOAD
    return;
#endif
    const int step = NW * rpw, last = nrows - 1;
    for (int r = wave * rpw + rl; r < nrows; r += 4 * step) {
        const int r1 = min(r + step, last), r2 = min(r + 2 * step, last), r3 = min(r + 3 * step, last);
        const hs_u32x4 v0 = hs_gload_off<hs_u32x4>(src0, (uint32_t)r * spitch + 16u * (uint32_t)q);
        const hs_u32x4 v1 = hs_gload_off<hs_u32x4>(src0, (uint32_t)r1 * spitch + 16u * (uint32_t)q);
        const hs_u32x4 v2 = hs_gload_off<hs_u32x4>(src0, (uint32_t)r2 * spitch + 16u * (uint32_t)q);
        const hs_u32x4 v3 = hs_gload_off<hs_u32x4>(src0, (uint32_t)r3 * spitch + 16u * (uint32_t)q);
        *reinterpret_cast<hs_u32x4*>(&s_dst[(uint32_t)r * dpitch + 16 * q]) = v0;
        *reinterpret_cast<hs_u32x4*>(&s_dst[(uint32_t)r1 * dpitch + 16 * q]) = v1;
        *reinterpret_cast<hs_u32x4*>(&s_dst[(uint32_t)r2 * dpitch + 16 * q]) = v2;
        *reinterpret_cast<hs_u32x4*>(&s_dst[(uint32_t)r3 * dpitch + 16 * q]) = v3;
    }
}

#define LT_ROWS 16
__global__ __launch_bounds__(256) void k_resize_level_lds(const HsLevel* __restrict__ lv, int level, HsImg0 img0, int lds_pitch, int lds_rows)
{
    extern __shared__ __attribute__((aligned(16))) uint8_t s_src[];
    uint16_t* const s_h = reinterpret_cast<uint16_t*>(s_src + (size_t)lds_pitch * lds_rows);
    const HsLevel& D = lv[level];
    const int img = blockIdx.z;
    const int tx = threadIdx.x & 63, ty = threadIdx.x >> 6;
    const int dx_tile = blockIdx.x * 256, dy_tile = blockIdx.y * LT_ROWS;

    const uint8_t* sbase; size_t spitch;
    if (level == 1) { sbase = hs_img0_ptr(img0, img); spitch = img0.row_stride; }
    else { const HsLevel& S = lv[level - 1]; sbase = S.base + (size_t)img * S.img_stride; spitch = S.pitch; }
    const int sw = lv[level - 1].w, sh = lv[level - 1].h;
    const HsXTab* xt = reinterpret_cast<const HsXTab*>(D.xofs);

    const int dy_last = min(dy_tile + LT_ROWS, D.h) - 1, dx_last = min(dx_tile + 256, D.w) - 1;
    const int sy_first = min(max(hs_cload_i16(D.yofs, dy_tile), 0), sh - 1);
    const int sy_last = min(max(hs_cload_i16(D.yofs, dy_last) + 1, 0), sh - 1);
    const int col0 = (int)(int16_t)hs_cload<uint32_t>(&xt[dx_tile]) & ~15;
    const int col_last = min((int)(int16_t)hs_cload<uint32_t>(&xt[dx_last]) + 1, sw - 1);
    const int nvec = ((col_last - col0) >> 4) + 1, nrow = sy_last - sy_first + 1;
    pyr_stage_source<4>(hs_uniform_ptr(sbase + (size_t)sy_first * spitch + col0), (uint32_t)spitch, s_src, (uint32_t)lds_pitch, nvec, nrow, threadIdx.x & 63, __builtin_amdgcn_readfirstlane(threadIdx.x >> 6));
    const int dx0 = dx_tile + 4 * tx;
    HsXTab t[4];
#pragma unroll
    for (int i = 0; i < 4; i++) t[i] = __builtin_bit_cast(HsXTab, hs_gload<uint64_t>(&xt[min(dx0 + i, D.w - 1)]));
    const int o0 = t[0].sx - col0;
    const int wbase = o0 & ~3, wshift = o0 & 3;
    uint32_t sel[4], coef[4];
#pragma unroll
    for (int i = 0; i < 4; i++) {
        const uint32_t q = (uint32_t)(t[i].sx - t[0].sx);
        sel[i] = q | 0x0c00u | ((q + 1) << 16) | 0x0c000000u;
        coef[i] = ((uint32_t)(uint16_t)t[i].a0 << 4) | ((uint32_t)(uint16_t)t[i].a1 << 20);
    }
    __syncthreads();
    for (int r = __builtin_amdgcn_readfirstlane(ty); r < nrow; r += 4) {
        const uint32_t* w = reinterpret_cast<const uint32_t*>(&s_src[r * lds_pitch + wbase]);
        const uint32_t d0 = w[0], d1 = w[1], d2 = w[2];
        const uint32_t wlo = __builtin_amdgcn_alignbyte(d1, d0, wshift), whi = __builtin_amdgcn_alignbyte(d2, d1, wshift);
        *reinterpret_cast<uint2*>(&s_h[r * 256 + 4 * tx]) = make_uint2(pyr_hpair(whi, wlo, sel[0], sel[1], coef[0], coef[1]), pyr_hpair(whi, wlo, sel[2], sel[3], coef[2], coef[3]));
    }
    __syncthreads();
    if (dx0 >= D.w) return;
    const int wave = __builtin_amdgcn_readfirstlane(threadIdx.x >> 6);
    uint8_t* const dimg = D.base + (size_t)img * D.img_stride;
    int sy4[LT_ROWS / 4]; uint32_t b4[LT_ROWS / 4];
#pragma unroll
    for (int rr = 0; rr < LT_ROWS / 4; rr++) { const int dy = min(dy_tile + wave + 4 * rr, D.h - 1); sy4[rr] = hs_cload_i16(D.yofs, dy); b4[rr] = hs_cload<uint32_t>(D.ibeta + 2 * dy); }
#pragma unroll
    for (int rr = 0; rr < LT_ROWS / 4; rr++) {
        const int dy = dy_tile + wave + 4 * rr;
        if (dy >= D.h) break;
        const int sy = sy4[rr];
        const uint32_t b01 = b4[rr];
        const uint32_t b0 = b01 & 0xFFFFu, b1 = b01 >> 16;
        const int r0 = min(max(sy, 0), sh - 1) - sy_first, r1 = min(max(sy + 1, 0), sh - 1) - sy_first;
        const uint2 H0 = *reinterpret_cast<const uint2*>(&s_h[r0 * 256 + 4 * tx]);
        const uint2 H1 = *reinterpret_cast<const uint2*>(&s_h[r1 * 256 + 4 * tx]);
        hs_gstore<uint32_t>(dimg + (size_t)dy * D.pitch + dx0, pyr_vquad(H0, H1, b0, b1));
    }
}

typedef uint32_t hs_u32x8 __attribute__((ext_vector_type(8)));
typedef uint32_t hs_u32x2 __attribute__((ext_vector_type(2)));
#ifndef FZ_ROWS
#define FZ_ROWS 16
#endif
#define FZ_APITCH 272
template <typename T> __device__ __forceinline__ void hs_gstore_off(uint8_t* uniform_base, uint32_t lane_off, T v)
{
    *(HS_GLOBAL T*)((HS_GLOBAL uint8_t*)(uintptr_t)uniform_base + lane_off) = v;
}
template <int NW>
__global__ __launch_bounds__(64 * NW) void k_resize_two_levels(HsPyrFuse F, HsImg0 img0)
{
    extern __shared__ __attribute__((aligned(16))) uint8_t smem[];
    const int TBX = F.tbx, lds_pitch = F.lds_pitch;
    uint8_t* const s_src = smem;
    uint8_t* const s_a = smem;
    uint16_t* const s_h = reinterpret_cast<uint16_t*>(smem + (size_t)lds_pitch * F.sr);
    const int img = blockIdx.z;
    const int tx = threadIdx.x & 63;
    const int wave = __builtin_amdgcn_readfirstlane(threadIdx.x >> 6);
    const HsPyrXTile X = __builtin_bit_cast(HsPyrXTile, hs_cload<hs_u32x8>(&F.xt[blockIdx.x]));
    const HsPyrYTile Y = __builtin_bit_cast(HsPyrYTile, hs_cload<hs_u32x8>(&F.yt[blockIdx.y]));
    const uint8_t* sbase; uint32_t spitch;
    if (F.sbase == nullptr) { sbase = hs_img0_ptr(img0, img); spitch = (uint32_t)img0.row_stride; }
    else { sbase = F.sbase + (size_t)img * F.s_img_stride; spitch = (uint32_t)F.spitch; }
    const int bx0 = blockIdx.x * TBX, by0 = blockIdx.y * FZ_ROWS;
    const int ax0 = X.ax0, ay0 = Y.ay0, nAr = Y.ay_last - Y.ay0 + 1, nSr = Y.n_sr, nvec = X.nvec;

    pyr_stage_source<NW>(hs_uniform_ptr(sbase + (size_t)Y.sy_first * spitch + X.col0), spitch, s_src, (uint32_t)lds_pitch, nvec, nSr, tx, wave);
    struct ColData { int wbase, wshift; uint32_t sel[4], coef[4]; };
    auto col_fetch = [&](const HsXTab* xt, int dx0, int wmax, uint64_t (&traw)[4]) {
#pragma unroll
        for (int i = 0; i < 4; i++) traw[i] = hs_gload<uint64_t>(&xt[min(dx0 + i, wmax)]);
    };
    auto col_data = [&](const uint64_t (&traw)[4], int origin) {
        HsXTab t[4];
#pragma unroll
        for (int i = 0; i < 4; i++) t[i] = __builtin_bit_cast(HsXTab, traw[i]);
        ColData c;
        const int o0 = t[0].sx - origin;
        c.wbase = o0 & ~3; c.wshift = o0 & 3;
#pragma unroll
        for (int i = 0; i < 4; i++) {
            const uint32_t q = (uint32_t)(t[i].sx - t[0].sx);
            c.sel[i] = q | 0x0c00u | ((q + 1) << 16) | 0x0c000000u;
            c.coef[i] = ((uint32_t)(uint16_t)t[i].a0 << 4) | ((uint32_t)(uint16_t)t[i].a1 << 20);
        }
        return c;
    };
    auto h_pass = [&](const uint8_t* src, int pitch, int nrow, const ColData& c) {
        for (int r = wave; r < nrow; r += NW) {
            const uint32_t* w = reinterpret_cast<const uint32_t*>(&src[r * pitch + c.wbase]);
            const uint32_t d0 = w[0], d1 = w[1], d2 = w[2];
            const uint32_t wlo = __builtin_amdgcn_alignbyte(d1, d0, c.wshift), whi = __builtin_amdgcn_alignbyte(d2, d1, c.wshift);
            *reinterpret_cast<uint2*>(&s_h[r * 256 + 4 * tx]) = make_uint2(pyr_hpair(whi, wlo, c.sel[0], c.sel[1], c.coef[0], c.coef[1]), pyr_hpair(whi, wlo, c.sel[2], c.sel[3], c.coef[2], c.coef[3]));
        }
    };
    const uint8_t* const h_lane = reinterpret_cast<const uint8_t*>(s_h) + 8 * tx;
    auto v_combine = [&](const HsPyrRow& rec) -> uint32_t {
        const uint2 H0 = *reinterpret_cast<const uint2*>(h_lane + rec.off0);
        const uint2 H1 = *reinterpret_cast<const uint2*>(h_lane + rec.off1);
        return pyr_vquad(H0, H1, rec.b0, rec.b1);
    };
    uint64_t tA[4], tB[4];
    col_fetch(F.xtA, ax0 + 4 * tx, F.aw - 1, tA);
    col_fetch(F.xtB, bx0 + 4 * tx, F.bw - 1, tB);
    const ColData cA = col_data(tA, X.col0);
    __syncthreads();
    h_pass(s_src, lds_pitch, nSr, cA);
    const ColData cB = col_data(tB, ax0);
    asm volatile("" :: "v"(cB.wbase), "v"(cB.wshift), "v"(cB.sel[0]), "v"(cB.sel[1]), "v"(cB.sel[2]), "v"(cB.sel[3]), "v"(cB.coef[0]), "v"(cB.coef[1]), "v"(cB.coef[2]), "v"(cB.coef[3]));
    __syncthreads();
    {
        uint8_t* const aimg = F.abase + (size_t)img * F.a_img_stride;
        const uint32_t acol = (uint32_t)(ax0 + 4 * tx);
        const bool own_col = (int)acol < X.own_x1;
        const HsPyrRow* recp = F.rowA + ((size_t)blockIdx.y * (uint32_t)F.slotA + (uint32_t)wave);
        HsPyrRow nxt = __builtin_bit_cast(HsPyrRow, hs_cload<hs_u32x2>(recp));
        uint8_t* rowp = aimg + (size_t)(ay0 + wave) * (uint32_t)F.apitch;
        const uint32_t rstep = (uint32_t)NW * (uint32_t)F.apitch;
        uint32_t* arow = reinterpret_cast<uint32_t*>(&s_a[wave * FZ_APITCH + 4 * tx]);
        const int own_k1 = Y.own_y1 - ay0;
        for (int k = wave; k < nAr; k += NW) {
            const HsPyrRow rec = nxt;
            recp += NW;
            nxt = __builtin_bit_cast(HsPyrRow, hs_cload<hs_u32x2>(recp));
            const uint32_t px = v_combine(rec);
            *arow = px;
            if (own_col && k < own_k1) hs_gstore_off<uint32_t>(rowp, acol, px);
            arow += NW * (FZ_APITCH / 4); rowp += rstep;
        }
    }
    __syncthreads();
    if (4 * tx < TBX) h_pass(s_a, FZ_APITCH, nAr, cB);
    __syncthreads();
    if (4 * tx < TBX && bx0 + 4 * tx < F.bw) {
        uint8_t* const bimg = F.bbase + (size_t)img * F.b_img_stride;
        const HsPyrRow* recp = F.rowB + ((size_t)blockIdx.y * (FZ_ROWS + 8) + (uint32_t)wave);
        HsPyrRow rec4[FZ_ROWS / NW];
#pragma unroll
        for (int rr = 0; rr < FZ_ROWS / NW; rr++) rec4[rr] = __builtin_bit_cast(HsPyrRow, hs_cload<hs_u32x2>(recp + NW * rr));
        uint8_t* rowp = bimg + (size_t)(by0 + wave) * (uint32_t)F.bpitch;
        const uint32_t rstep = (uint32_t)NW * (uint32_t)F.bpitch;
#pragma unroll
        for (int rr = 0; rr < FZ_ROWS / NW; rr++) {
            const int by = by0 + wave + NW * rr;
            if (by >= F.bh) break;
            hs_gstore_off<uint32_t>(rowp, (uint32_t)(bx0 + 4 * tx), v_combine(rec4[rr]));
            rowp += rstep;
        }
    }
}

#ifdef HS_PYR_PROFILE
__device__ unsigned long long g_pyr_prof[64];
__device__ unsigned long long g_pyr_wg[4096 * 2];
extern "C" void hs_debug_pyr_profile(unsigned long long* out64) { (void)hipDeviceSynchronize(); (void)hipMemcpyFromSymbol(out64, HIP_SYMBOL(g_pyr_prof), sizeof(unsigned long long) * 64); }
extern "C" void hs_debug_pyr_workgroups(unsigned long long* out8192) { (void)hipDeviceSynchronize(); (void)hipMemcpyFromSymbol(out8192, HIP_SYMBOL(g_pyr_wg), sizeof(unsigned long long) * 8192); }
#define PYR_MARK() do { if (threadIdx.x == 0 && blockIdx.x == gridDim.x / 2 && blockIdx.y == gridDim.y / 2 && blockIdx.z == 0 && pk < 62) g_pyr_prof[pk++] = __builtin_amdgcn_s_memtime(); } while (0)
#else
#define PYR_MARK()
#endif
template <int NW>
__global__ __launch_bounds__(64 * NW) void k_resize_chain(HsPyrChain F, HsImg0 img0)
{
#ifdef HS_PYR_PROFILE
    int pk = 0;
    const unsigned pyr_wg = (blockIdx.z * gridDim.y + blockIdx.y) * gridDim.x + blockIdx.x;
    if (threadIdx.x == 0 && pyr_wg < 4096) g_pyr_wg[2 * pyr_wg] = __builtin_amdgcn_s_memrealtime();
#endif
    PYR_MARK();
    extern __shared__ __attribute__((aligned(16))) uint8_t smem[];
    uint8_t* const s_x = smem;
    uint16_t* const s_h = reinterpret_cast<uint16_t*>(smem + F.x_bytes);
    const int img = blockIdx.z;
    const int tx = threadIdx.x & 63;
    const int wave = __builtin_amdgcn_readfirstlane(threadIdx.x >> 6);
    const uint8_t* sbase; uint32_t spitch;
    if (F.sbase == nullptr) { sbase = hs_img0_ptr(img0, img); spitch = (uint32_t)img0.row_stride; }
    else { sbase = F.sbase + (size_t)img * F.s_img_stride; spitch = (uint32_t)F.spitch; }
    int src_pitch = F.lds_pitch;
    auto ld_x = [&](int st) { return __builtin_bit_cast(HsPyrStageX, hs_cload<hs_u32x8>(&F.st[st].tx[blockIdx.x])); };
    auto ld_y = [&](int st) { return __builtin_bit_cast(HsPyrStageY, hs_cload<hs_u32x8>(&F.st[st].ty[blockIdx.y])); };
    auto ld_t = [&](int st, const HsPyrStageX& X, uint64_t (&t)[4]) {
        const HsPyrStage& S = F.st[st];
#pragma unroll
        for (int i = 0; i < 4; i++) t[i] = hs_gload<uint64_t>(&S.xt[min(X.x0 + 4 * tx + i, S.w - 1)]);
    };
    HsPyrStageX X = ld_x(0); HsPyrStageY Y = ld_y(0);
    uint64_t traw[4]; ld_t(0, X, traw);
    for (int st = 0; st < F.nstage; st++) {
        const HsPyrStage& S = F.st[st];
        const int stn = min(st + 1, F.nstage - 1);
        const HsPyrStageX Xn = ld_x(stn); const HsPyrStageY Yn = ld_y(stn);
        if (st == 0) pyr_stage_source<NW>(hs_uniform_ptr(sbase + (size_t)Y.src_y0 * spitch + X.src_x0), spitch, s_x, (uint32_t)src_pitch, X.nvec, Y.n_src, tx, wave);
        int wbase, wshift; uint32_t sel[4], coef[4];
        {
            HsXTab t[4];
#pragma unroll
            for (int i = 0; i < 4; i++) t[i] = __builtin_bit_cast(HsXTab, traw[i]);
            const int o0 = t[0].sx - X.src_x0;
            wbase = o0 & ~3; wshift = o0 & 3;
#pragma unroll
            for (int i = 0; i < 4; i++) {
                const uint32_t q = (uint32_t)(t[i].sx - t[0].sx);
                sel[i] = q | 0x0c00u | ((q + 1) << 16) | 0x0c000000u;
                coef[i] = ((uint32_t)(uint16_t)t[i].a0 << 4) | ((uint32_t)(uint16_t)t[i].a1 << 20);
            }
        }
        __syncthreads();
        PYR_MARK();
        if (4 * tx < X.ncols) {
            for (int r = wave; r < Y.n_src; r += 2 * NW) {
                const bool two = r + NW < Y.n_src;
                const uint32_t* wa = reinterpret_cast<const uint32_t*>(&s_x[r * src_pitch + wbase]);
                const uint32_t* wb = reinterpret_cast<const uint32_t*>(&s_x[(two ? r + NW : r) * src_pitch + wbase]);
                const uint32_t a0 = wa[0], a1 = wa[1], a2 = wa[2], b0 = wb[0], b1 = wb[1], b2 = wb[2];
                const uint32_t alo = __builtin_amdgcn_alignbyte(a1, a0, wshift), ahi = __builtin_amdgcn_alignbyte(a2, a1, wshift);
                const uint32_t blo = __builtin_amdgcn_alignbyte(b1, b0, wshift), bhi = __builtin_amdgcn_alignbyte(b2, b1, wshift);
                *reinterpret_cast<uint2*>(&s_h[r * 256 + 4 * tx]) = make_uint2(pyr_hpair(ahi, alo, sel[0], sel[1], coef[0], coef[1]), pyr_hpair(ahi, alo, sel[2], sel[3], coef[2], coef[3]));
                if (two) *reinterpret_cast<uint2*>(&s_h[(r + NW) * 256 + 4 * tx]) = make_uint2(pyr_hpair(bhi, blo, sel[0], sel[1], coef[0], coef[1]), pyr_hpair(bhi, blo, sel[2], sel[3], coef[2], coef[3]));
            }
        }
        ld_t(stn, Xn, traw);
        __syncthreads();
        PYR_MARK();
        {
            uint8_t* const dimg = S.base + (size_t)img * S.img_stride;
            const uint32_t col = (uint32_t)(X.x0 + 4 * tx);
            const bool lane_on = 4 * tx < X.ncols, own_col = (int)col < X.own_x1;
            const bool keep = st + 1 < F.nstage;
            const HsPyrRow* recp = S.rows + ((size_t)blockIdx.y * (uint32_t)S.slot + (uint32_t)wave);
            HsPyrRow nxt0 = __builtin_bit_cast(HsPyrRow, hs_cload<hs_u32x2>(recp)), nxt1 = __builtin_bit_cast(HsPyrRow, hs_cload<hs_u32x2>(recp + NW));
            const uint8_t* const h_lane = reinterpret_cast<const uint8_t*>(s_h) + 8 * tx;
            uint8_t* rowp = dimg + (size_t)(Y.y0 + wave) * (uint32_t)S.pitch;
            const uint32_t rstep = (uint32_t)NW * (uint32_t)S.pitch;
            uint32_t* xrow = reinterpret_cast<uint32_t*>(&s_x[wave * FZ_APITCH + 4 * tx]);
            for (int y = Y.y0 + wave; y <= Y.y_last; y += 2 * NW) {
                const HsPyrRow rec0 = nxt0, rec1 = nxt1;
                recp += 2 * NW;
                nxt0 = __builtin_bit_cast(HsPyrRow, hs_cload<hs_u32x2>(recp)); nxt1 = __builtin_bit_cast(HsPyrRow, hs_cload<hs_u32x2>(recp + NW));
                const bool two = y + NW <= Y.y_last;
                if (lane_on) {
                    const uint2 A0 = *reinterpret_cast<const uint2*>(h_lane + rec0.off0), A1 = *reinterpret_cast<const uint2*>(h_lane + rec0.off1);
                    const uint2 B0 = *reinterpret_cast<const uint2*>(h_lane + rec1.off0), B1 = *reinterpret_cast<const uint2*>(h_lane + rec1.off1);
                    const uint32_t pa = pyr_vquad(A0, A1, rec0.b0, rec0.b1), pb = pyr_vquad(B0, B1, rec1.b0, rec1.b1);
                    if (keep) { *xrow = pa; if (two) xrow[NW * (FZ_APITCH / 4)] = pb; }
                    if (own_col && y < Y.own_y1) hs_gstore_off<uint32_t>(rowp, col, pa);
                    if (own_col && two && y + NW < Y.own_y1) hs_gstore_off<uint32_t>(rowp + rstep, col, pb);
                }
                xrow += 2 * NW * (FZ_APITCH / 4); rowp += 2 * rstep;
            }
        }
        src_pitch = FZ_APITCH;
        X = Xn; Y = Yn;
        PYR_MARK();
    }
#ifdef HS_PYR_PROFILE
    if (threadIdx.x == 0 && blockIdx.x == gridDim.x / 2 && blockIdx.y == gridDim.y / 2 && blockIdx.z == 0) g_pyr_prof[63] = pk;
    __syncthreads();
    if (threadIdx.x == 0 && pyr_wg < 4096) g_pyr_wg[2 * pyr_wg + 1] = __builtin_amdgcn_s_memrealtime();
#endif
}

void hs_pyramid_plan_chain(const HsLevel* h_lv, int first, int n, const int16_t* const* xtab, const int16_t* const* yofs, const int16_t* const* ibeta,
                           std::vector<uint64_t>& blob, HsPyrChain& C, size_t lds_max, int tile_rows)
{
    C = HsPyrChain{};
    if (tile_rows <= 0) tile_rows = FZ_ROWS;
    if (n < 2 || n > HS_PYR_CHAIN_MAX || first < 1) return;
    auto clampi = [](int v, int lo, int hi) { return v < lo ? lo : (v > hi ? hi : v); };
    for (int i = 0; i < n; i++) {
        const HsLevel& D = h_lv[first + i]; const HsLevel& S = h_lv[first + i - 1];
        if ((double)S.w / D.w > 2.0 || (double)S.h / D.h > 2.0 || D.w < 8 || D.h < 1) return;
    }
    const HsLevel& LAST = h_lv[first + n - 1];
    const int nby = (LAST.h + tile_rows - 1) / tile_rows;
    std::vector<std::vector<HsPyrStageY>> ty(n, std::vector<HsPyrStageY>(nby));
    int h_rows = 0, x_rows0 = 0, x_rows = 0;
    for (int by = 0; by < nby; by++) {
        int y0 = by * tile_rows;
        for (int i = n - 1; i >= 0; i--) {
            ty[i][by] = HsPyrStageY{};
            ty[i][by].y0 = y0;
            if (i > 0) y0 = by == 0 ? 0 : clampi(yofs[first + i][y0], 0, h_lv[first + i - 1].h - 1);
        }
    }
    for (int by = 0; by < nby; by++)
        for (int i = n - 1; i >= 0; i--) {
            HsPyrStageY& t = ty[i][by];
            t.own_y1 = by + 1 < nby ? ty[i][by + 1].y0 : h_lv[first + i].h;
            if (t.own_y1 < t.y0) return;
        }
    for (int by = 0; by < nby; by++) {
        int need_last = std::min(by * tile_rows + tile_rows, LAST.h) - 1;
        for (int i = n - 1; i >= 0; i--) {
            const HsLevel& S = h_lv[first + i - 1];
            const int16_t* yo = yofs[first + i];
            HsPyrStageY& t = ty[i][by];
            t.y_last = std::max(need_last, t.own_y1 - 1);
            const int src_first = clampi(yo[t.y0], 0, S.h - 1), src_last = clampi(yo[t.y_last] + 1, 0, S.h - 1);
            if (i > 0) {
                if (src_first < ty[i - 1][by].y0) return;
                t.src_y0 = ty[i - 1][by].y0;
                need_last = src_last;
            } else {
                t.src_y0 = src_first; t.n_src = src_last - src_first + 1;
                x_rows0 = std::max(x_rows0, t.n_src);
                h_rows = std::max(h_rows, t.n_src);
            }
        }
        for (int i = n - 1; i >= 1; i--) {
            ty[i][by].n_src = ty[i - 1][by].y_last - ty[i - 1][by].y0 + 1;
            x_rows = std::max(x_rows, ty[i][by].n_src);
            h_rows = std::max(h_rows, ty[i][by].n_src);
        }
    }
    std::vector<std::vector<HsPyrStageX>> best_txs; int best_tbx = 0, best_pitch = 0; size_t best_xbytes = 0;
    for (int tbx = 256; tbx >= 64; tbx -= 4) {
        const int nbx = (LAST.w + tbx - 1) / tbx;
        std::vector<std::vector<HsPyrStageX>> txs(n, std::vector<HsPyrStageX>(nbx));
        bool ok = true; int pitch = 0;
        for (int bx = 0; bx < nbx && ok; bx++) {
            int x0 = bx * tbx;
            for (int i = n - 1; i >= 0; i--) {
                txs[i][bx] = HsPyrStageX{};
                txs[i][bx].x0 = x0;
                if (i > 0) x0 = bx == 0 ? 0 : (xtab[first + i][4 * x0] & ~3);
            }
        }
        for (int bx = 0; bx < nbx && ok; bx++)
            for (int i = n - 1; i >= 0; i--) {
                const HsLevel& D = h_lv[first + i];
                HsPyrStageX& t = txs[i][bx];
                t.own_x1 = bx + 1 < nbx ? txs[i][bx + 1].x0 : ((D.w + 3) & ~3);
                if (t.own_x1 < t.x0) ok = false;
            }
        for (int bx = 0; bx < nbx && ok; bx++) {
            int need_last = std::min(bx * tbx + tbx, LAST.w) - 1;
            for (int i = n - 1; i >= 0; i--) {
                const HsLevel& D = h_lv[first + i]; const HsLevel& S = h_lv[first + i - 1];
                HsPyrStageX& t = txs[i][bx];
                const int reg_last = std::max(need_last, std::min(t.own_x1, D.w) - 1);
                t.ncols = ((std::max(reg_last + 1, t.own_x1) - t.x0) + 3) & ~3;
                if (t.ncols > 256 || t.ncols <= 0) { ok = false; break; }
                const int16_t* xt = xtab[first + i];
                const int src_need_first = xt[4 * t.x0], src_need_last = std::min(xt[4 * std::min(reg_last, D.w - 1)] + 1, S.w - 1);
                if (i > 0) {
                    const HsPyrStageX& u = txs[i - 1][bx];
                    if (src_need_first < u.x0) { ok = false; break; }
                    t.src_x0 = u.x0;
                    const int lastlane_col = std::min(t.x0 + t.ncols - 4, D.w - 1);
                    if (xt[4 * lastlane_col] - u.x0 + 12 > FZ_APITCH) { ok = false; break; }
                    need_last = src_need_last;
                } else {
                    t.src_x0 = src_need_first & ~15;
                    t.nvec = ((src_need_last - t.src_x0) >> 4) + 1;
                    pitch = std::max(pitch, t.nvec * 16 + 16);
                    const int lastlane_col = std::min(t.x0 + t.ncols - 4, D.w - 1);
                    if (xt[4 * lastlane_col] - t.src_x0 + 12 > t.nvec * 16 + 16) { ok = false; break; }
                }
            }
        }
        if (!ok) continue;
        pitch = (pitch + 15) & ~15;
        const size_t x_bytes = std::max((size_t)pitch * x_rows0, (size_t)FZ_APITCH * x_rows);
        const size_t lds = ((x_bytes + 15) & ~(size_t)15) + (size_t)h_rows * 256 * 2;
        if (lds > lds_max || h_rows > 127 || x_rows > 127) continue;
        best_tbx = tbx; best_pitch = pitch; best_xbytes = x_bytes; best_txs = txs;
        break;
    }
    if (best_tbx == 0) return;
    {
        const int tbx = best_tbx, pitch = best_pitch, nbx = (LAST.w + tbx - 1) / tbx;
        const size_t x_bytes = best_xbytes;
        const std::vector<std::vector<HsPyrStageX>>& txs = best_txs;
        if (blob.empty()) blob.push_back(0);
        C.sbase = first == 1 ? nullptr : h_lv[first - 1].base; C.s_img_stride = h_lv[first - 1].img_stride; C.spitch = h_lv[first - 1].pitch; C.nstage = n;
        for (int i = 0; i < n; i++) {
            const HsLevel& D = h_lv[first + i];
            HsPyrStage& S = C.st[i];
            S.base = D.base; S.img_stride = D.img_stride; S.pitch = D.pitch; S.w = D.w; S.h = D.h;
            S.xt = reinterpret_cast<const HsXTab*>(D.xofs);
            int slot = 0;
            for (int by = 0; by < nby; by++) slot = std::max(slot, ty[i][by].y_last - ty[i][by].y0 + 1);
            slot += 4 * 8;
            const size_t orow = blob.size(); blob.resize(orow + (size_t)slot * nby);
            const int sh = h_lv[first + i - 1].h;
            for (int by = 0; by < nby; by++) {
                const HsPyrStageY& t = ty[i][by];
                for (int k = 0; k < slot; k++) {
                    const int dy = std::min(t.y0 + k, t.y_last);
                    HsPyrRow r;
                    r.off0 = (uint16_t)((clampi(yofs[first + i][dy], 0, sh - 1) - t.src_y0) * 512);
                    r.off1 = (uint16_t)((clampi(yofs[first + i][dy] + 1, 0, sh - 1) - t.src_y0) * 512);
                    r.b0 = (uint16_t)ibeta[first + i][2 * dy]; r.b1 = (uint16_t)ibeta[first + i][2 * dy + 1];
                    memcpy(&blob[orow + (size_t)by * slot + k], &r, 8);
                }
            }
            S.rows = reinterpret_cast<const HsPyrRow*>(orow * 8); S.slot = slot;
            const size_t ox = blob.size(); blob.resize(ox + 4 * (size_t)nbx);
            memcpy(&blob[ox], txs[i].data(), 32 * (size_t)nbx);
            const size_t oy = blob.size(); blob.resize(oy + 4 * (size_t)nby);
            memcpy(&blob[oy], ty[i].data(), 32 * (size_t)nby);
            S.tx = reinterpret_cast<const HsPyrStageX*>(ox * 8); S.ty = reinterpret_cast<const HsPyrStageY*>(oy * 8);
        }
        C.tbx = tbx; C.lds_pitch = pitch; C.x_bytes = (int32_t)((x_bytes + 15) & ~(size_t)15); C.h_rows = h_rows; C.grid_x = nbx; C.grid_y = nby; C.valid = 1;
    }
}

void hs_pyramid_build_tables(const HsLevel* h_lv, int nlevels, const int16_t* const* xtab, const int16_t* const* yofs, const int16_t* const* ibeta,
                             std::vector<uint64_t>& blob, std::vector<HsPyrFuse>& fuse)
{
    fuse.assign(nlevels, HsPyrFuse{});
    auto clampi = [](int v, int lo, int hi) { return v < lo ? lo : (v > hi ? hi : v); };
    if (blob.empty()) blob.push_back(0);
    for (int l = 1; l + 1 < nlevels; l++) {
        const HsLevel& A = h_lv[l];
        if (A.fuse_tbx <= 0) continue;
        const HsLevel& B = h_lv[l + 1]; const HsLevel& S = h_lv[l - 1];
        const int16_t* xA = xtab[l]; const int16_t* xB = xtab[l + 1]; const int16_t* yA = yofs[l]; const int16_t* yB = yofs[l + 1];
        const int tbx = A.fuse_tbx, nbx = (B.w + tbx - 1) / tbx, nby = (B.h + FZ_ROWS - 1) / FZ_ROWS;
        HsPyrFuse& F = fuse[l];
        F.sbase = l == 1 ? nullptr : S.base; F.s_img_stride = S.img_stride; F.spitch = S.pitch;
        F.abase = A.base; F.a_img_stride = A.img_stride; F.apitch = A.pitch; F.aw = A.w; F.ah = A.h;
        F.bbase = B.base; F.b_img_stride = B.img_stride; F.bpitch = B.pitch; F.bw = B.w; F.bh = B.h;
        F.xtA = reinterpret_cast<const HsXTab*>(A.xofs); F.xtB = reinterpret_cast<const HsXTab*>(B.xofs);
        F.tbx = tbx; F.sr = A.fuse_sr; F.lds_pitch = A.fuse_pitch; F.valid = 1;
        const size_t ox = blob.size(); blob.resize(ox + 4 * (size_t)nbx);
        for (int bx = 0; bx < nbx; bx++) {
            const int bx0 = bx * tbx; const bool last_x = bx0 + tbx >= B.w;
            HsPyrXTile t{};
            t.ax0 = bx == 0 ? 0 : (xB[4 * bx0] & ~3);
            t.own_x1 = last_x ? ((A.w + 3) & ~3) : (xB[4 * (bx0 + tbx)] & ~3);
            const int ax_lastcol = std::min(t.ax0 + 255, A.w - 1);
            t.col0 = xA[4 * t.ax0] & ~15;
            const int col_last = std::min(xA[4 * ax_lastcol] + 1, S.w - 1);
            t.nvec = ((col_last - t.col0) >> 4) + 1;
            memcpy(&blob[ox + 4 * (size_t)bx], &t, 32);
        }
        const size_t oy = blob.size(); blob.resize(oy + 4 * (size_t)nby);
        for (int by = 0; by < nby; by++) {
            const int by0 = by * FZ_ROWS, by_last = std::min(by0 + FZ_ROWS, B.h) - 1; const bool last_y = by0 + FZ_ROWS >= B.h;
            HsPyrYTile t{};
            t.ay0 = by == 0 ? 0 : clampi(yB[by0], 0, A.h - 1);
            t.own_y1 = last_y ? A.h : clampi(yB[by0 + FZ_ROWS], 0, A.h - 1);
            t.ay_last = std::max(clampi(yB[by_last] + 1, 0, A.h - 1), t.own_y1 - 1);
            t.sy_first = clampi(yA[t.ay0], 0, S.h - 1);
            t.n_sr = clampi(yA[t.ay_last] + 1, 0, S.h - 1) - t.sy_first + 1;
            memcpy(&blob[oy + 4 * (size_t)by], &t, 32);
        }
        F.xt = reinterpret_cast<const HsPyrXTile*>(ox * 8); F.yt = reinterpret_cast<const HsPyrYTile*>(oy * 8);
        const int slotA = A.fuse_ar + 8, slotB = FZ_ROWS + 8;
        const size_t oa = blob.size(); blob.resize(oa + (size_t)slotA * nby);
        const size_t ob = blob.size(); blob.resize(ob + (size_t)slotB * nby);
        for (int by = 0; by < nby; by++) {
            HsPyrYTile t; memcpy(&t, &blob[oy + 4 * (size_t)by], 32);
            const int by0 = by * FZ_ROWS;
            for (int k = 0; k < slotA; k++) {
                const int ay = std::min(t.ay0 + k, t.ay_last);
                HsPyrRow r;
                r.off0 = (uint16_t)((clampi(yA[ay], 0, S.h - 1) - t.sy_first) * 512); r.off1 = (uint16_t)((clampi(yA[ay] + 1, 0, S.h - 1) - t.sy_first) * 512);
                r.b0 = (uint16_t)ibeta[l][2 * ay]; r.b1 = (uint16_t)ibeta[l][2 * ay + 1];
                memcpy(&blob[oa + (size_t)by * slotA + k], &r, 8);
            }
            for (int k = 0; k < slotB; k++) {
                const int y = std::min(by0 + k, B.h - 1);
                HsPyrRow r;
                r.off0 = (uint16_t)((clampi(yB[y], 0, A.h - 1) - t.ay0) * 512); r.off1 = (uint16_t)((clampi(yB[y] + 1, 0, A.h - 1) - t.ay0) * 512);
                r.b0 = (uint16_t)ibeta[l + 1][2 * y]; r.b1 = (uint16_t)ibeta[l + 1][2 * y + 1];
                memcpy(&blob[ob + (size_t)by * slotB + k], &r, 8);
            }
        }
        F.rowA = reinterpret_cast<const HsPyrRow*>(oa * 8); F.rowB = reinterpret_cast<const HsPyrRow*>(ob * 8); F.slotA = slotA;
    }
}

void hs_pyramid_plan_fusion(HsLevel* h_lv, int nlevels, const int16_t* const* xtab, const int16_t* const* yofs, int tbx_max)
{
    for (int l = 1; l < nlevels; l++) h_lv[l].fuse_tbx = h_lv[l].fuse_ar = h_lv[l].fuse_sr = h_lv[l].fuse_pitch = 0;
    for (int l = 1; l + 1 < nlevels; l += 2) {
        HsLevel& A = h_lv[l]; const HsLevel& B = h_lv[l + 1]; const HsLevel& S = h_lv[l - 1];
        const double scxA = (double)S.w / A.w, scyA = (double)S.h / A.h, scxB = (double)A.w / B.w, scyB = (double)A.h / B.h;
        if (scxA > 2.0 || scxB > 2.0 || scyA > 2.0 || scyB > 2.0 || B.w < 8 || B.h < 1) continue;
        int tbx = std::min(256, ((int)(250.0 / scxB)) & ~3);
        if (tbx_max >= 64) tbx = std::min(tbx, tbx_max & ~3);
        if (tbx < 64) continue;
        const int16_t* xA = xtab[l]; const int16_t* xB = xtab[l + 1]; const int16_t* yA = yofs[l]; const int16_t* yB = yofs[l + 1];
        auto clampi = [](int v, int lo, int hi) { return v < lo ? lo : (v > hi ? hi : v); };
        int ar = 0, sr = 0, pitch = 0; bool ok = true;
        for (int by0 = 0; by0 < B.h && ok; by0 += FZ_ROWS) {
            const int by_last = std::min(by0 + FZ_ROWS, B.h) - 1; const bool last_y = by0 + FZ_ROWS >= B.h;
            const int ay0 = by0 == 0 ? 0 : clampi(yB[by0], 0, A.h - 1);
            const int own_y1 = last_y ? A.h : clampi(yB[by0 + FZ_ROWS], 0, A.h - 1);
            const int ay_last = std::max(clampi(yB[by_last] + 1, 0, A.h - 1), own_y1 - 1);
            if (own_y1 <= ay0 && !last_y) {  }
            if (clampi(yB[by0], 0, A.h - 1) < ay0) ok = false;
            ar = std::max(ar, ay_last - ay0 + 1);
            const int sy_first = clampi(yA[ay0], 0, S.h - 1), sy_last = clampi(yA[ay_last] + 1, 0, S.h - 1);
            sr = std::max(sr, sy_last - sy_first + 1);
        }
        for (int bx0 = 0; bx0 < B.w && ok; bx0 += tbx) {
            const int bx_last = std::min(bx0 + tbx, B.w) - 1; const bool last_x = bx0 + tbx >= B.w;
            const int ax0 = bx0 == 0 ? 0 : (xB[4 * bx0] & ~3);
            const int own_x1 = last_x ? ((A.w + 3) & ~3) : (xB[4 * (bx0 + tbx)] & ~3);
            const int need_last = std::min(xB[4 * bx_last] + 1, A.w - 1);
            if (xB[4 * bx0] < ax0 || own_x1 - ax0 > 256 || need_last - ax0 > 255 || own_x1 < ax0) ok = false;
            if (xB[4 * std::min(bx0 + tbx - 4, B.w - 1)] - ax0 + 12 > FZ_APITCH) ok = false;
            const int ax_lastcol = std::min(ax0 + 255, A.w - 1);
            const int col0 = xA[4 * ax0] & ~15, col_last = std::min(xA[4 * ax_lastcol] + 1, S.w - 1);
            pitch = std::max(pitch, ((col_last - col0) >> 4) * 16 + 16 + 16);
            if (xA[4 * ax0] < col0) ok = false;
        }
        if (!ok) continue;
        pitch = (pitch + 15) & ~15;
        const size_t lds = (size_t)pitch * sr + (size_t)std::max(sr, ar) * 256 * 2;
        if ((size_t)FZ_APITCH * ar > (size_t)pitch * sr || lds > 60 * 1024) continue;
        A.fuse_tbx = tbx; A.fuse_ar = ar; A.fuse_sr = sr; A.fuse_pitch = pitch;
    }
}

static int pyr_nw8_wg_per_cu()
{
    static int v = [] { const char* e = getenv("HS_PYRAMID_NW8"); return e ? atoi(e) : 3; }();
    return v;
}
int hs_launch_pyramid(const HsLevel* d_lv, const HsLevel* h_lv, const HsPyrFuse* fuse, const HsPyrChain* chain, int nlevels, HsImg0 img0, int batch, hipStream_t s, const HsPyrChain* deep)
{
    const bool big_lds = deep != nullptr && [] {
        int dev = -1;
        if (hipGetDevice(&dev) != hipSuccess || dev < 0 || dev >= 64) { (void)hipGetLastError(); return false; }
        static std::atomic<int8_t> state[64];
        const int8_t st = state[dev].load(std::memory_order_acquire);
        if (st) return st == 1;
        const bool ok = hipFuncSetAttribute(reinterpret_cast<const void*>(&k_resize_chain<8>), hipFuncAttributeMaxDynamicSharedMemorySize, HS_PYR_DEEP_LDS) == hipSuccess &&
                        hipFuncSetAttribute(reinterpret_cast<const void*>(&k_resize_chain<4>), hipFuncAttributeMaxDynamicSharedMemorySize, HS_PYR_DEEP_LDS) == hipSuccess;
        if (!ok) (void)hipGetLastError();
        state[dev].store(ok ? 1 : 2, std::memory_order_release);
        return ok;
    }();
    int n_launches = 0;
    for (int l = 1; l < nlevels; l++, n_launches++) {
        const HsLevel& D = h_lv[l];
        if (deep && deep[l].valid && l + deep[l].nstage <= nlevels) {
            bool vec16 = true;
            if (l == 1) vec16 = (((uintptr_t)img0.base | (uintptr_t)img0.base2 | img0.row_stride | img0.img_stride) & 15) == 0 && ((h_lv[0].w + 15) & ~15) <= (int)img0.row_stride;
            const HsPyrChain& C = deep[l];
            const size_t lds = (size_t)C.x_bytes + (size_t)C.h_rows * 256 * 2;
            if (vec16 && (lds <= 64 * 1024 || big_lds)) {
                dim3 grid(C.grid_x, C.grid_y, batch);
                if ((size_t)grid.x * grid.y * grid.z <= (size_t)256 * pyr_nw8_wg_per_cu()) hipLaunchKernelGGL(k_resize_chain<8>, grid, dim3(512), lds, s, C, img0);
                else hipLaunchKernelGGL(k_resize_chain<4>, grid, dim3(256), lds, s, C, img0);
                l += C.nstage - 1;
                continue;
            }
        }
        if (chain && D.chain_n > 0 && chain[l].valid && l + D.chain_n <= nlevels) {
            bool vec16 = true;
            if (l == 1) vec16 = (((uintptr_t)img0.base | (uintptr_t)img0.base2 | img0.row_stride | img0.img_stride) & 15) == 0 && ((h_lv[0].w + 15) & ~15) <= (int)img0.row_stride;
            if (vec16) {
                const HsPyrChain& C = chain[l];
                const size_t lds = (size_t)C.x_bytes + (size_t)C.h_rows * 256 * 2;
                dim3 grid(C.grid_x, C.grid_y, batch);
                if ((size_t)grid.x * grid.y * grid.z <= (size_t)256 * pyr_nw8_wg_per_cu()) hipLaunchKernelGGL(k_resize_chain<8>, grid, dim3(512), lds, s, C, img0);
                else hipLaunchKernelGGL(k_resize_chain<4>, grid, dim3(256), lds, s, C, img0);
                l += C.nstage - 1;
                continue;
            }
        }
        if (D.fuse_tbx > 0 && l + 1 < nlevels && fuse && fuse[l].valid) {
            bool vec16 = true;
            if (l == 1) vec16 = (((uintptr_t)img0.base | (uintptr_t)img0.base2 | img0.row_stride | img0.img_stride) & 15) == 0 && ((h_lv[0].w + 15) & ~15) <= (int)img0.row_stride;
            if (vec16) {
                const HsLevel& B = h_lv[l + 1];
                const size_t lds = (size_t)D.fuse_pitch * D.fuse_sr + (size_t)std::max(D.fuse_sr, D.fuse_ar) * 256 * 2;
                dim3 grid((B.w + D.fuse_tbx - 1) / D.fuse_tbx, (B.h + FZ_ROWS - 1) / FZ_ROWS, batch);
                if ((size_t)grid.x * grid.y * grid.z <= (size_t)256 * pyr_nw8_wg_per_cu()) hipLaunchKernelGGL(k_resize_two_levels<8>, grid, dim3(512), lds, s, fuse[l], img0);
                else hipLaunchKernelGGL(k_resize_two_levels<4>, grid, dim3(256), lds, s, fuse[l], img0);
                l++;
                continue;
            }
        }
        const int sw = h_lv[l - 1].w, sh = h_lv[l - 1].h;
        bool vec16 = true;
        if (l == 1) vec16 = (((uintptr_t)img0.base | (uintptr_t)img0.base2 | img0.row_stride | img0.img_stride) & 15) == 0 && ((sw + 15) & ~15) <= (int)img0.row_stride;
        const double scx = (double)sw / D.w, scy = (double)sh / D.h;
        const int lds_pitch = (((int)(256 * scx) + 2 + 15 + 15) & ~15) + 16;
        const int lds_rows = (int)(LT_ROWS * scy) + 4;
        const size_t lds_bytes = (size_t)lds_pitch * lds_rows + (size_t)lds_rows * 256 * 2;
        if (vec16 && lds_bytes <= 60 * 1024 && scx <= 2.0) {
            dim3 grid((D.w + 255) / 256, (D.h + LT_ROWS - 1) / LT_ROWS, batch);
            hipLaunchKernelGGL(k_resize_level_lds, grid, dim3(256), lds_bytes, s, d_lv, l, img0, lds_pitch, lds_rows);
            continue;
        }
        dim3 block(64, 4, 1);
        dim3 grid((D.w + 255) / 256, (D.h + 3) / 4, batch);
        bool aligned = true;
        if (l == 1) aligned = (((uintptr_t)img0.base | (uintptr_t)img0.base2 | img0.row_stride | img0.img_stride) & 3) == 0;
        if (aligned) hipLaunchKernelGGL(k_resize_level<true>, grid, block, 0, s, d_lv, l, img0);
        else hipLaunchKernelGGL(k_resize_level<false>, grid, block, 0, s, d_lv, l, img0);
    }
    return n_launches;
}

int hs_pyramid_launch_count(const HsLevel* h_lv, int nlevels)
{
    int n = 0;
    for (int l = 1; l < nlevels; l++) { n++; if (h_lv[l].chain_n > 0 && l + h_lv[l].chain_n <= nlevels) l += h_lv[l].chain_n - 1; else if (h_lv[l].fuse_tbx > 0 && l + 1 < nlevels) l++; }
    return n;
}

__global__ __launch_bounds__(256) void k_copy_u32(uint32_t* __restrict__ d, const uint32_t* __restrict__ s, size_t n)
{
    for (size_t i = (size_t)blockIdx.x * 256 + threadIdx.x; i < n; i += (size_t)gridDim.x * 256) d[i] = s[i];
}
__global__ __launch_bounds__(256) void k_copy_u128(uint4* __restrict__ d, const uint4* __restrict__ s, size_t n)
{
    for (size_t i = (size_t)blockIdx.x * 256 + threadIdx.x; i < n; i += (size_t)gridDim.x * 256) d[i] = s[i];
}
__global__ __launch_bounds__(256) void k_copy_u128x4(uint4* __restrict__ d_, const uint4* __restrict__ s_, size_t n)
{
    hs_u32x4* const d = reinterpret_cast<hs_u32x4*>(d_);
    const hs_u32x4* const s = reinterpret_cast<const hs_u32x4*>(s_);
    const size_t stride = (size_t)gridDim.x * 1024;
    size_t i = (size_t)blockIdx.x * 1024 + threadIdx.x;
    for (; i + 768 < n; i += stride) {
        const hs_u32x4 a = __builtin_nontemporal_load(s + i), b = __builtin_nontemporal_load(s + i + 256), c = __builtin_nontemporal_load(s + i + 512), e = __builtin_nontemporal_load(s + i + 768);
        __builtin_nontemporal_store(a, d + i); __builtin_nontemporal_store(b, d + i + 256); __builtin_nontemporal_store(c, d + i + 512); __builtin_nontemporal_store(e, d + i + 768);
    }
    for (int k = 0; k < 4; k++) if (i + 256 * k < n) d[i + 256 * k] = s[i + 256 * k];
}
void hs_launch_stream_copy(void* d_dst, const void* d_src, size_t bytes, int width, hipStream_t s)
{
    if (width == 64) { hipLaunchKernelGGL(k_copy_u128x4, dim3(4096), dim3(256), 0, s, (uint4*)d_dst, (const uint4*)d_src, bytes / 16); return; }
    if (width == 4) hipLaunchKernelGGL(k_copy_u32, dim3(2048), dim3(256), 0, s, (uint32_t*)d_dst, (const uint32_t*)d_src, bytes / 4);
    else hipLaunchKernelGGL(k_copy_u128, dim3(2048), dim3(256), 0, s, (uint4*)d_dst, (const uint4*)d_src, bytes / 16);
}
```

Measured before the change: 48590.

## Precompute per-tile horizontal resize column records at plan time

Adds a plan-time pass that bakes the per-thread horizontal interpolation records (word base, shift, byte-select masks, packed coefficients) for every pyramid tile into a device blob. The resize kernels (single level, two-level fused, chain) then load these with three coalesced vector loads instead of gathering four xtab entries and rebuilding the selectors in registers. This cuts scalar/ALU setup and dependent gathers per workgroup, at the cost of extra device memory and a larger per-tile record load.

```diff
diff --git a/hyslam_amd/csrc/hs_api.hip b/hyslam_amd/csrc/hs_api.hip
--- a/hyslam_amd/csrc/hs_api.hip
+++ b/hyslam_amd/csrc/hs_api.hip
@@ -91,6 +91,9 @@
         bool keys_dirty = false;
         HsBuf<uint8_t> d_pyr_tabs;
         std::vector<HsPyrFuse> pyr_fuse;
+        HsBuf<uint8_t> d_pyr_cols;
+        std::vector<HsPyrFuseCols> pyr_fuse_cols; std::vector<HsPyrChainCols> pyr_chain_cols, pyr_deep_cols;
+        std::vector<const uint8_t*> pyr_level_cols;
         std::vector<HsPyrChain> pyr_deep;
         std::vector<HsPyrChain> pyr_chain;
         HsBuf<uint2> d_cand; HsBuf<uint32_t> d_pts_xy, d_pts_sk; HsBuf<uint16_t> d_pt_node;
@@ -172,6 +175,10 @@
         relocate(F.abase, g.d_pyr.p); relocate(F.bbase, g.d_pyr.p); relocate(F.xtA, g.d_tables.p); relocate(F.xtB, g.d_tables.p);
         relocate(F.rowA, g.d_pyr_tabs.p); relocate(F.rowB, g.d_pyr_tabs.p); relocate(F.xt, g.d_pyr_tabs.p); relocate(F.yt, g.d_pyr_tabs.p);
     }
+    for (HsPyrFuseCols& K : g.pyr_fuse_cols) { if (K.a) relocate(K.a, g.d_pyr_cols.p); if (K.b) relocate(K.b, g.d_pyr_cols.p); }
+    for (std::vector<HsPyrChainCols>* plan : { &g.pyr_chain_cols, &g.pyr_deep_cols })
+        for (HsPyrChainCols& K : *plan) for (const uint8_t*& c : K.st) if (c) relocate(c, g.d_pyr_cols.p);
+    for (size_t l = 1; l < g.pyr_level_cols.size(); l++) relocate(g.pyr_level_cols[l], g.d_pyr_cols.p);
 }
 template <class T, class V> hipError_t upload(const HsBuf<T>& d, const std::vector<V>& v)
 {
@@ -203,6 +210,8 @@
     g.qhist_stride = P.qhist_stride; g.qbest_stride = P.qbest_stride; g.plan_digest = P.digest;
     g.lv = std::move(P.lv); g.lv_n = std::move(P.lv_n);
     g.pyr_fuse = std::move(P.pyr_fuse); g.pyr_chain = std::move(P.pyr_chain); g.pyr_deep = std::move(P.pyr_deep);
+    g.pyr_fuse_cols = std::move(P.pyr_fuse_cols); g.pyr_chain_cols = std::move(P.pyr_chain_cols); g.pyr_deep_cols = std::move(P.pyr_deep_cols);
+    g.pyr_level_cols = std::move(P.pyr_level_cols);
 
     HIP_TRY(h, g.d_pyr.grow(std::max<size_t>(P.pyr_per_img * batch, 256)));
     HIP_TRY(h, g.d_tables.grow(std::max<size_t>(P.tables.size(), 256 / sizeof(int16_t))));
@@ -223,6 +232,7 @@
     HIP_TRY(h, g.d_qhist.grow(std::max<size_t>((size_t)g.qhist_stride * batch, 256 / 4)));
     HIP_TRY(h, g.d_qbest.grow(std::max<size_t>((size_t)g.qbest_stride * batch, 256 / 8)));
     HIP_TRY(h, g.d_pyr_tabs.grow(std::max<size_t>(P.pyr_tabs.size() * 8, 256)));
+    HIP_TRY(h, g.d_pyr_cols.grow(std::max<size_t>(P.pyr_cols.size() * 8, 256)));
     HIP_TRY(h, g.d_fast_items.grow(P.items.size()));
     HIP_TRY(h, g.d_fast_items_n.grow(P.items_n.size()));
     HIP_TRY(h, g.d_fast_ovf.grow(std::max<size_t>(hs_fast_overflow_bytes(g.max_hcell, std::max(g.fast_items, g.fast_items_n) * batch, h->fast_knobs), 256) / 4));
@@ -238,6 +248,7 @@
     HIP_TRY(h, upload(g.d_qkeys, P.qkeys));
     HIP_TRY(h, upload(g.d_fast_qt, P.fast_qt));
     HIP_TRY(h, upload(g.d_pyr_tabs, P.pyr_tabs));
+    HIP_TRY(h, upload(g.d_pyr_cols, P.pyr_cols));
     HIP_TRY(h, hipMemcpy(h->d_lv, g.lv.data(), sizeof(HsLevel) * L, hipMemcpyHostToDevice));
     HIP_TRY(h, hipMemcpy(h->d_lv + L, g.lv_n.data(), sizeof(HsLevel) * L, hipMemcpyHostToDevice));
     HIP_TRY(h, upload(g.d_fast_items, P.items));
@@ -383,14 +394,14 @@
         if (rc != HS_OK) return rc;
         quadtree(0, 1, h->s_aux);
         HIP_TRY(h, hipEventRecord(h->ev_sjoin, h->s_aux));
-        h->geo.last_pyr_launches = hs_launch_pyramid(h->d_lv, h->geo.lv.data(), g.pyr_fuse.data(), g.pyr_chain.data(), L, img0, batch, s, deep);
+        h->geo.last_pyr_launches = hs_launch_pyramid(h->d_lv, h->geo.lv.data(), g.pyr_fuse.data(), g.pyr_chain.data(), L, img0, batch, s, HsPyrCols{ g.pyr_fuse_cols.data(), g.pyr_chain_cols.data(), g.pyr_deep_cols.data(), g.pyr_level_cols.data() }, deep);
         rc = fast(0, n_items - items0, 0, s);
         if (rc != HS_OK) return rc;
         quadtree(1, L - 1, s);
         HIP_TRY(h, hipStreamWaitEvent(s, h->ev_sjoin, 0));
     } else {
         mark(h, 0, s);
-        h->geo.last_pyr_launches = hs_launch_pyramid(h->d_lv, h->geo.lv.data(), g.pyr_fuse.data(), g.pyr_chain.data(), L, img0, batch, s, deep);
+        h->geo.last_pyr_launches = hs_launch_pyramid(h->d_lv, h->geo.lv.data(), g.pyr_fuse.data(), g.pyr_chain.data(), L, img0, batch, s, HsPyrCols{ g.pyr_fuse_cols.data(), g.pyr_chain_cols.data(), g.pyr_deep_cols.data(), g.pyr_level_cols.data() }, deep);
         mark(h, 1, s);
         const int rc = fast(0, n_items, 0, s);
         if (rc != HS_OK) return rc;
@@ -476,6 +487,14 @@
     for (int l = 0; l < L; l++) out[4] += h->geo.lv[l].qt_hist_off != 0xFFFFFFFFu;
     out[5] = longest; out[6] = lds;
     if (L > 1 && !h->geo.pyr_deep.empty() && h->geo.pyr_deep[1].valid) out[7] = h->geo.pyr_deep[1].grid_x * h->geo.pyr_deep[1].grid_y;
+}
+void hs_debug_pyramid_plan(const hs_orb* h, HsDebugPyramidPlan* out)
+{
+    *out = HsDebugPyramidPlan{};
+    if (!h || h->geo.w <= 0) return;
+    out->nlevels = h->p.nlevels; out->lv = h->geo.lv.data();
+    out->fuse = h->geo.pyr_fuse.data(); out->chain = h->geo.pyr_chain.data(); out->deep = h->geo.pyr_deep.data();
+    out->cols = HsPyrCols{ h->geo.pyr_fuse_cols.data(), h->geo.pyr_chain_cols.data(), h->geo.pyr_deep_cols.data(), h->geo.pyr_level_cols.data() };
 }
 uint64_t hs_debug_plan_digest(const hs_orb* h) { return h && h->geo.w > 0 ? h->geo.plan_digest : 0; }
 
diff --git a/hyslam_amd/csrc/hs_internal.h b/hyslam_amd/csrc/hs_internal.h
--- a/hyslam_amd/csrc/hs_internal.h
+++ b/hyslam_amd/csrc/hs_internal.h
@@ -122,6 +122,8 @@
 struct HsPyrYTile { int32_t ay0, own_y1, ay_last, sy_first, n_sr, _r[3]; };
 struct HsPyrRow { uint16_t off0, off1, b0, b1; };
 static_assert(sizeof(HsPyrXTile) == 32 && sizeof(HsPyrYTile) == 32 && sizeof(HsPyrRow) == 8, "scalar-load records");
+struct HsPyrCol { int32_t wbase, wshift; uint32_t sel[4], coef[4]; };
+#define HS_PYR_COL_TILE_BYTES 3072
 struct HsPyrFuse {
     const uint8_t* sbase;
     uint64_t s_img_stride; int32_t spitch; int32_t _r0;
@@ -150,6 +152,10 @@
     int32_t grid_x, grid_y, valid, _r;
 };
 
+struct HsPyrFuseCols { const uint8_t* a; const uint8_t* b; };
+struct HsPyrChainCols { const uint8_t* st[HS_PYR_CHAIN_MAX]; };
+struct HsPyrCols { const HsPyrFuseCols* fuse; const HsPyrChainCols* chain; const HsPyrChainCols* deep; const uint8_t* const* level; };
+
 #define HS_STRIP_ENTRY_BYTES 16
 #define HS_STRIP_SHIFT 5
 struct __attribute__((aligned(16))) HsStripEntry { float uR; int32_t octave; uint32_t idx_band; uint32_t _pad; };
@@ -159,11 +165,17 @@
 inline int hs_stereo_strips(int n_rows) { return (n_rows > 0 ? ((n_rows - 1) >> 5) : 0) + 1; }
 
 int  hs_launch_pyramid(const HsLevel* d_lv, const HsLevel* h_lv, const HsPyrFuse* fuse , const HsPyrChain* chain , int nlevels, HsImg0 img0, int batch, hipStream_t s,
+                       const HsPyrCols& cols ,
                        const HsPyrChain* deep = nullptr );
+struct hs_orb;
+struct HsDebugPyramidPlan { int nlevels; const HsLevel* lv; const HsPyrFuse* fuse; const HsPyrChain* chain; const HsPyrChain* deep; HsPyrCols cols; };
+void hs_debug_pyramid_plan(const hs_orb* h, HsDebugPyramidPlan* out);
+size_t hs_pyramid_col_records(const int16_t* xt , int w, int x0, int origin, std::vector<uint64_t>& blob);
+size_t hs_pyramid_level_cols(const int16_t* xt, int w, std::vector<uint64_t>& blob);
 void hs_pyramid_plan_chain(const HsLevel* h_lv, int first, int n, const int16_t* const* xtab, const int16_t* const* yofs, const int16_t* const* ibeta,
-                           std::vector<uint64_t>& blob, HsPyrChain& C, size_t lds_max = 60 * 1024, int tile_rows = 0 );
+                           std::vector<uint64_t>& blob, HsPyrChain& C, std::vector<uint64_t>& cols_blob, HsPyrChainCols& CC , size_t lds_max = 60 * 1024, int tile_rows = 0 );
 void hs_pyramid_build_tables(const HsLevel* h_lv, int nlevels, const int16_t* const* xtab, const int16_t* const* yofs, const int16_t* const* ibeta,
-                             std::vector<uint64_t>& blob, std::vector<HsPyrFuse>& fuse);
+                             std::vector<uint64_t>& blob, std::vector<HsPyrFuse>& fuse, std::vector<uint64_t>& cols_blob, std::vector<HsPyrFuseCols>& fuse_cols );
 void hs_pyramid_plan_fusion(HsLevel* h_lv, int nlevels, const int16_t* const* xtab , const int16_t* const* yofs , int tbx_max = 0 );
 int hs_pyramid_launch_count(const HsLevel* h_lv, int nlevels);
 int hs_fast_group_cells(int wcell, int ncols, int lc);
diff --git a/hyslam_amd/csrc/hs_plan.h b/hyslam_amd/csrc/hs_plan.h
--- a/hyslam_amd/csrc/hs_plan.h
+++ b/hyslam_amd/csrc/hs_plan.h
@@ -29,9 +29,13 @@
     std::vector<uint16_t> qkeys;
     std::vector<HsFastQt> fast_qt;
     std::vector<uint64_t> pyr_tabs;
+    std::vector<uint64_t> pyr_cols;
+    std::vector<HsPyrFuseCols> pyr_fuse_cols;
+    std::vector<HsPyrChainCols> pyr_chain_cols, pyr_deep_cols;
     std::vector<HsPyrFuse> pyr_fuse;
     std::vector<HsPyrChain> pyr_chain;
     std::vector<HsPyrChain> pyr_deep;
+    std::vector<const uint8_t*> pyr_level_cols;
     std::vector<HsFastItem> items, items_n;
     uint64_t digest = 0;
 };
diff --git a/hyslam_amd/csrc/hs_plan.hip b/hyslam_amd/csrc/hs_plan.hip
--- a/hyslam_amd/csrc/hs_plan.hip
+++ b/hyslam_amd/csrc/hs_plan.hip
@@ -162,15 +162,16 @@
     hs_pyramid_plan_fusion(lv.data(), L, xt.data(), yo.data(), k.pyr_tbx_max);
     if (k.no_fuse) for (int l = 0; l < L; l++) lv[l].fuse_tbx = 0;
     std::vector<uint64_t>& blob = P.pyr_tabs;
-    hs_pyramid_build_tables(lv.data(), L, xt.data(), yo.data(), ib.data(), blob, P.pyr_fuse);
-    P.pyr_chain.assign(L, HsPyrChain{});
+    std::vector<uint64_t>& cblob = P.pyr_cols;
+    hs_pyramid_build_tables(lv.data(), L, xt.data(), yo.data(), ib.data(), blob, P.pyr_fuse, cblob, P.pyr_fuse_cols);
+    P.pyr_chain.assign(L, HsPyrChain{}); P.pyr_chain_cols.assign(L, HsPyrChainCols{});
     for (int l = 0; l < L; l++) lv[l].chain_n = 0;
     if (!k.no_fuse && k.chain_mode != 0) {
         if (k.chain_mode == 2) {
             for (int l = 1; l + 1 < L; l += 2) {
                 int n = (l + 3 == L) ? 3 : 2;
-                hs_pyramid_plan_chain(lv.data(), l, n, xt.data(), yo.data(), ib.data(), blob, P.pyr_chain[l]);
-                if (!P.pyr_chain[l].valid && n == 3) hs_pyramid_plan_chain(lv.data(), l, 2, xt.data(), yo.data(), ib.data(), blob, P.pyr_chain[l]);
+                hs_pyramid_plan_chain(lv.data(), l, n, xt.data(), yo.data(), ib.data(), blob, P.pyr_chain[l], cblob, P.pyr_chain_cols[l]);
+                if (!P.pyr_chain[l].valid && n == 3) hs_pyramid_plan_chain(lv.data(), l, 2, xt.data(), yo.data(), ib.data(), blob, P.pyr_chain[l], cblob, P.pyr_chain_cols[l]);
                 if (P.pyr_chain[l].valid) { lv[l].chain_n = P.pyr_chain[l].nstage; if (P.pyr_chain[l].nstage == 3) l++; }
             }
         } else if (k.pyr_plan_set) {
@@ -179,7 +180,7 @@
             for (const char* q = k.pyr_plan.c_str(); *q && l < L; ) {
                 const int n = std::min(atoi(q), L - l);
                 if (n >= 3 || (n == 2 && (chain2 || !(l & 1)))) {
-                    hs_pyramid_plan_chain(lv.data(), l, n, xt.data(), yo.data(), ib.data(), blob, P.pyr_chain[l], HS_PYR_DEEP_LDS, 0);
+                    hs_pyramid_plan_chain(lv.data(), l, n, xt.data(), yo.data(), ib.data(), blob, P.pyr_chain[l], cblob, P.pyr_chain_cols[l], HS_PYR_DEEP_LDS, 0);
                     if (P.pyr_chain[l].valid) lv[l].chain_n = n;
                 }
                 if (n == 1) lv[l].fuse_tbx = 0;
@@ -189,16 +190,18 @@
             }
         } else if (L >= 4 && ((L - 1) & 1)) {
             const int l = L - 3;
-            hs_pyramid_plan_chain(lv.data(), l, 3, xt.data(), yo.data(), ib.data(), blob, P.pyr_chain[l]);
+            hs_pyramid_plan_chain(lv.data(), l, 3, xt.data(), yo.data(), ib.data(), blob, P.pyr_chain[l], cblob, P.pyr_chain_cols[l]);
             if (P.pyr_chain[l].valid) lv[l].chain_n = 3;
         }
     }
-    P.pyr_deep.assign(L, HsPyrChain{});
+    P.pyr_level_cols.assign(L, nullptr);
+    for (int l = 1; l < L; l++) P.pyr_level_cols[l] = at_offset<uint8_t>(hs_pyramid_level_cols(xt[l], lv[l].w, cblob));
+    P.pyr_deep.assign(L, HsPyrChain{}); P.pyr_deep_cols.assign(L, HsPyrChainCols{});
     if (!k.no_fuse && k.deep_max_batch > 0) {
         for (int l = 1; l + 1 < L;) {
             int took = 0;
             for (int n = std::min(HS_PYR_CHAIN_MAX, L - l); n >= 2 && !took; n--) {
-                hs_pyramid_plan_chain(lv.data(), l, n, xt.data(), yo.data(), ib.data(), blob, P.pyr_deep[l], HS_PYR_DEEP_LDS, k.deep_rows);
+                hs_pyramid_plan_chain(lv.data(), l, n, xt.data(), yo.data(), ib.data(), blob, P.pyr_deep[l], cblob, P.pyr_deep_cols[l], HS_PYR_DEEP_LDS, k.deep_rows);
                 if (P.pyr_deep[l].valid) took = n;
             }
             l += took ? took : 1;
diff --git a/hyslam_amd/csrc/kernels_pyramid.hip b/hyslam_amd/csrc/kernels_pyramid.hip
--- a/hyslam_amd/csrc/kernels_pyramid.hip
+++ b/hyslam_amd/csrc/kernels_pyramid.hip
@@ -96,6 +96,25 @@
     asm("v_pk_lshrrev_b16 %0, %2, %1" : "=v"(a2) : "v"(a), "v"(two));
     asm("v_pk_lshrrev_b16 %0, %2, %1" : "=v"(c2) : "v"(c), "v"(two));
     return __builtin_amdgcn_perm(c2, a2, 0x06040200u);
+}
+
+typedef uint32_t hs_u32x2 __attribute__((ext_vector_type(2)));
+struct PyrColRaw { hs_u32x4 p0, p1; hs_u32x2 p2; };
+__device__ __forceinline__ PyrColRaw pyr_col_request(const uint8_t* cols , uint32_t tile_col, int tx)
+{
+    const uint8_t* const tile = cols + (size_t)tile_col * HS_PYR_COL_TILE_BYTES;
+    const uint32_t off = 16u * (uint32_t)tx;
+    PyrColRaw r;
+    r.p0 = hs_gload_off<hs_u32x4>(tile, off); r.p1 = hs_gload_off<hs_u32x4>(tile, off + 1024u); r.p2 = hs_gload_off<hs_u32x2>(tile, off + 2048u);
+    return r;
+}
+__device__ __forceinline__ HsPyrCol pyr_col_data(const PyrColRaw& r)
+{
+    HsPyrCol c;
+    c.wbase = (int)r.p0.x; c.wshift = (int)r.p0.y;
+    c.sel[0] = r.p0.z; c.sel[1] = r.p0.w; c.sel[2] = r.p1.x; c.sel[3] = r.p1.y;
+    c.coef[0] = r.p1.z; c.coef[1] = r.p1.w; c.coef[2] = r.p2.x; c.coef[3] = r.p2.y;
+    return c;
 }
 
 template <int NW>
@@ -122,7 +141,7 @@
 }
 
 #define LT_ROWS 16
-__global__ __launch_bounds__(256) void k_resize_level_lds(const HsLevel* __restrict__ lv, int level, HsImg0 img0, int lds_pitch, int lds_rows)
+__global__ __launch_bounds__(256) void k_resize_level_lds(const HsLevel* __restrict__ lv, int level, HsImg0 img0, int lds_pitch, int lds_rows, const uint8_t* cols )
 {
     extern __shared__ __attribute__((aligned(16))) uint8_t s_src[];
     uint16_t* const s_h = reinterpret_cast<uint16_t*>(s_src + (size_t)lds_pitch * lds_rows);
@@ -145,24 +164,13 @@
     const int nvec = ((col_last - col0) >> 4) + 1, nrow = sy_last - sy_first + 1;
     pyr_stage_source<4>(hs_uniform_ptr(sbase + (size_t)sy_first * spitch + col0), (uint32_t)spitch, s_src, (uint32_t)lds_pitch, nvec, nrow, threadIdx.x & 63, __builtin_amdgcn_readfirstlane(threadIdx.x >> 6));
     const int dx0 = dx_tile + 4 * tx;
-    HsXTab t[4];
-#pragma unroll
-    for (int i = 0; i < 4; i++) t[i] = __builtin_bit_cast(HsXTab, hs_gload<uint64_t>(&xt[min(dx0 + i, D.w - 1)]));
-    const int o0 = t[0].sx - col0;
-    const int wbase = o0 & ~3, wshift = o0 & 3;
-    uint32_t sel[4], coef[4];
-#pragma unroll
-    for (int i = 0; i < 4; i++) {
-        const uint32_t q = (uint32_t)(t[i].sx - t[0].sx);
-        sel[i] = q | 0x0c00u | ((q + 1) << 16) | 0x0c000000u;
-        coef[i] = ((uint32_t)(uint16_t)t[i].a0 << 4) | ((uint32_t)(uint16_t)t[i].a1 << 20);
-    }
+    const HsPyrCol c = pyr_col_data(pyr_col_request(cols, blockIdx.x, tx));
     __syncthreads();
     for (int r = __builtin_amdgcn_readfirstlane(ty); r < nrow; r += 4) {
-        const uint32_t* w = reinterpret_cast<const uint32_t*>(&s_src[r * lds_pitch + wbase]);
+        const uint32_t* w = reinterpret_cast<const uint32_t*>(&s_src[r * lds_pitch + c.wbase]);
         const uint32_t d0 = w[0], d1 = w[1], d2 = w[2];
-        const uint32_t wlo = __builtin_amdgcn_alignbyte(d1, d0, wshift), whi = __builtin_amdgcn_alignbyte(d2, d1, wshift);
-        *reinterpret_cast<uint2*>(&s_h[r * 256 + 4 * tx]) = make_uint2(pyr_hpair(whi, wlo, sel[0], sel[1], coef[0], coef[1]), pyr_hpair(whi, wlo, sel[2], sel[3], coef[2], coef[3]));
+        const uint32_t wlo = __builtin_amdgcn_alignbyte(d1, d0, c.wshift), whi = __builtin_amdgcn_alignbyte(d2, d1, c.wshift);
+        *reinterpret_cast<uint2*>(&s_h[r * 256 + 4 * tx]) = make_uint2(pyr_hpair(whi, wlo, c.sel[0], c.sel[1], c.coef[0], c.coef[1]), pyr_hpair(whi, wlo, c.sel[2], c.sel[3], c.coef[2], c.coef[3]));
     }
     __syncthreads();
     if (dx0 >= D.w) return;
@@ -186,7 +194,6 @@
 }
 
 typedef uint32_t hs_u32x8 __attribute__((ext_vector_type(8)));
-typedef uint32_t hs_u32x2 __attribute__((ext_vector_type(2)));
 #ifndef FZ_ROWS
 #define FZ_ROWS 16
 #endif
@@ -196,7 +203,7 @@
     *(HS_GLOBAL T*)((HS_GLOBAL uint8_t*)(uintptr_t)uniform_base + lane_off) = v;
 }
 template <int NW>
-__global__ __launch_bounds__(64 * NW) void k_resize_two_levels(HsPyrFuse F, HsImg0 img0)
+__global__ __launch_bounds__(64 * NW) void k_resize_two_levels(HsPyrFuse F, HsImg0 img0, HsPyrFuseCols K)
 {
     extern __shared__ __attribute__((aligned(16))) uint8_t smem[];
     const int TBX = F.tbx, lds_pitch = F.lds_pitch;
@@ -215,27 +222,7 @@
     const int ax0 = X.ax0, ay0 = Y.ay0, nAr = Y.ay_last - Y.ay0 + 1, nSr = Y.n_sr, nvec = X.nvec;
 
     pyr_stage_source<NW>(hs_uniform_ptr(sbase + (size_t)Y.sy_first * spitch + X.col0), spitch, s_src, (uint32_t)lds_pitch, nvec, nSr, tx, wave);
-    struct ColData { int wbase, wshift; uint32_t sel[4], coef[4]; };
-    auto col_fetch = [&](const HsXTab* xt, int dx0, int wmax, uint64_t (&traw)[4]) {
-#pragma unroll
-        for (int i = 0; i < 4; i++) traw[i] = hs_gload<uint64_t>(&xt[min(dx0 + i, wmax)]);
-    };
-    auto col_data = [&](const uint64_t (&traw)[4], int origin) {
-        HsXTab t[4];
-#pragma unroll
-        for (int i = 0; i < 4; i++) t[i] = __builtin_bit_cast(HsXTab, traw[i]);
-        ColData c;
-        const int o0 = t[0].sx - origin;
-        c.wbase = o0 & ~3; c.wshift = o0 & 3;
-#pragma unroll
-        for (int i = 0; i < 4; i++) {
-            const uint32_t q = (uint32_t)(t[i].sx - t[0].sx);
-            c.sel[i] = q | 0x0c00u | ((q + 1) << 16) | 0x0c000000u;
-            c.coef[i] = ((uint32_t)(uint16_t)t[i].a0 << 4) | ((uint32_t)(uint16_t)t[i].a1 << 20);
-        }
-        return c;
-    };
-    auto h_pass = [&](const uint8_t* src, int pitch, int nrow, const ColData& c) {
+    auto h_pass = [&](const uint8_t* src, int pitch, int nrow, const HsPyrCol& c) {
         for (int r = wave; r < nrow; r += NW) {
             const uint32_t* w = reinterpret_cast<const uint32_t*>(&src[r * pitch + c.wbase]);
             const uint32_t d0 = w[0], d1 = w[1], d2 = w[2];
@@ -249,13 +236,11 @@
         const uint2 H1 = *reinterpret_cast<const uint2*>(h_lane + rec.off1);
         return pyr_vquad(H0, H1, rec.b0, rec.b1);
     };
-    uint64_t tA[4], tB[4];
-    col_fetch(F.xtA, ax0 + 4 * tx, F.aw - 1, tA);
-    col_fetch(F.xtB, bx0 + 4 * tx, F.bw - 1, tB);
-    const ColData cA = col_data(tA, X.col0);
+    const PyrColRaw rA = pyr_col_request(K.a, blockIdx.x, tx), rB = pyr_col_request(K.b, blockIdx.x, tx);
+    const HsPyrCol cA = pyr_col_data(rA);
     __syncthreads();
     h_pass(s_src, lds_pitch, nSr, cA);
-    const ColData cB = col_data(tB, ax0);
+    const HsPyrCol cB = pyr_col_data(rB);
     asm volatile("" :: "v"(cB.wbase), "v"(cB.wshift), "v"(cB.sel[0]), "v"(cB.sel[1]), "v"(cB.sel[2]), "v"(cB.sel[3]), "v"(cB.coef[0]), "v"(cB.coef[1]), "v"(cB.coef[2]), "v"(cB.coef[3]));
     __syncthreads();
     {
@@ -309,7 +294,7 @@
 #define PYR_MARK()
 #endif
 template <int NW>
-__global__ __launch_bounds__(64 * NW) void k_resize_chain(HsPyrChain F, HsImg0 img0)
+__global__ __launch_bounds__(64 * NW) void k_resize_chain(HsPyrChain F, HsImg0 img0, HsPyrChainCols K)
 {
 #ifdef HS_PYR_PROFILE
     int pk = 0;
@@ -329,32 +314,17 @@
     int src_pitch = F.lds_pitch;
     auto ld_x = [&](int st) { return __builtin_bit_cast(HsPyrStageX, hs_cload<hs_u32x8>(&F.st[st].tx[blockIdx.x])); };
     auto ld_y = [&](int st) { return __builtin_bit_cast(HsPyrStageY, hs_cload<hs_u32x8>(&F.st[st].ty[blockIdx.y])); };
-    auto ld_t = [&](int st, const HsPyrStageX& X, uint64_t (&t)[4]) {
-        const HsPyrStage& S = F.st[st];
-#pragma unroll
-        for (int i = 0; i < 4; i++) t[i] = hs_gload<uint64_t>(&S.xt[min(X.x0 + 4 * tx + i, S.w - 1)]);
-    };
+    auto ld_c = [&](int st) { return pyr_col_request(K.st[st], blockIdx.x, tx); };
     HsPyrStageX X = ld_x(0); HsPyrStageY Y = ld_y(0);
-    uint64_t traw[4]; ld_t(0, X, traw);
+    PyrColRaw craw = ld_c(0);
     for (int st = 0; st < F.nstage; st++) {
         const HsPyrStage& S = F.st[st];
         const int stn = min(st + 1, F.nstage - 1);
         const HsPyrStageX Xn = ld_x(stn); const HsPyrStageY Yn = ld_y(stn);
         if (st == 0) pyr_stage_source<NW>(hs_uniform_ptr(sbase + (size_t)Y.src_y0 * spitch + X.src_x0), spitch, s_x, (uint32_t)src_pitch, X.nvec, Y.n_src, tx, wave);
-        int wbase, wshift; uint32_t sel[4], coef[4];
-        {
-            HsXTab t[4];
-#pragma unroll
-            for (int i = 0; i < 4; i++) t[i] = __builtin_bit_cast(HsXTab, traw[i]);
-            const int o0 = t[0].sx - X.src_x0;
-            wbase = o0 & ~3; wshift = o0 & 3;
-#pragma unroll
-            for (int i = 0; i < 4; i++) {
-                const uint32_t q = (uint32_t)(t[i].sx - t[0].sx);
-                sel[i] = q | 0x0c00u | ((q + 1) << 16) | 0x0c000000u;
-                coef[i] = ((uint32_t)(uint16_t)t[i].a0 << 4) | ((uint32_t)(uint16_t)t[i].a1 << 20);
-            }
-        }
+        const HsPyrCol c = pyr_col_data(craw);
+        const int wbase = c.wbase, wshift = c.wshift;
+        const uint32_t (&sel)[4] = c.sel, (&coef)[4] = c.coef;
         __syncthreads();
         PYR_MARK();
         if (4 * tx < X.ncols) {
@@ -369,7 +339,7 @@
                 if (two) *reinterpret_cast<uint2*>(&s_h[(r + NW) * 256 + 4 * tx]) = make_uint2(pyr_hpair(bhi, blo, sel[0], sel[1], coef[0], coef[1]), pyr_hpair(bhi, blo, sel[2], sel[3], coef[2], coef[3]));
             }
         }
-        ld_t(stn, Xn, traw);
+        craw = ld_c(stn);
         __syncthreads();
         PYR_MARK();
         {
@@ -410,10 +380,44 @@
 #endif
 }
 
+size_t hs_pyramid_col_records(const int16_t* xt, int w, int x0, int origin, std::vector<uint64_t>& blob)
+{
+    if (blob.empty()) blob.push_back(0);
+    if (blob.size() & 1) blob.push_back(0);
+    const size_t o = blob.size(); blob.resize(o + HS_PYR_COL_TILE_BYTES / 8, 0);
+    uint32_t* const out = reinterpret_cast<uint32_t*>(&blob[o]);
+    for (int t = 0; t < 64; t++) {
+        const int16_t* e[4];
+        for (int i = 0; i < 4; i++) e[i] = xt + 4 * (size_t)std::min(x0 + 4 * t + i, w - 1);
+        HsPyrCol c;
+        const int o0 = e[0][0] - origin;
+        c.wbase = o0 & ~3; c.wshift = o0 & 3;
+        for (int i = 0; i < 4; i++) {
+            const uint32_t q = (uint32_t)(e[i][0] - e[0][0]);
+            c.sel[i] = q | 0x0c00u | ((q + 1) << 16) | 0x0c000000u;
+            c.coef[i] = ((uint32_t)(uint16_t)e[i][1] << 4) | ((uint32_t)(uint16_t)e[i][2] << 20);
+        }
+        uint32_t* const p0 = out + 4 * t, * const p1 = out + 256 + 4 * t, * const p2 = out + 512 + 4 * t;
+        p0[0] = (uint32_t)c.wbase; p0[1] = (uint32_t)c.wshift; p0[2] = c.sel[0]; p0[3] = c.sel[1];
+        p1[0] = c.sel[2]; p1[1] = c.sel[3]; p1[2] = c.coef[0]; p1[3] = c.coef[1];
+        p2[0] = c.coef[2]; p2[1] = c.coef[3];
+    }
+    return o * 8;
+}
+size_t hs_pyramid_level_cols(const int16_t* xt, int w, std::vector<uint64_t>& blob)
+{
+    size_t first = 0;
+    for (int x0 = 0; x0 < w; x0 += 256) {
+        const size_t o = hs_pyramid_col_records(xt, w, x0, xt[4 * (size_t)x0] & ~15, blob);
+        if (x0 == 0) first = o;
+    }
+    return first;
+}
+
 void hs_pyramid_plan_chain(const HsLevel* h_lv, int first, int n, const int16_t* const* xtab, const int16_t* const* yofs, const int16_t* const* ibeta,
-                           std::vector<uint64_t>& blob, HsPyrChain& C, size_t lds_max, int tile_rows)
-{
-    C = HsPyrChain{};
+                           std::vector<uint64_t>& blob, HsPyrChain& C, std::vector<uint64_t>& cols_blob, HsPyrChainCols& CC, size_t lds_max, int tile_rows)
+{
+    C = HsPyrChain{}; CC = HsPyrChainCols{};
     if (tile_rows <= 0) tile_rows = FZ_ROWS;
     if (n < 2 || n > HS_PYR_CHAIN_MAX || first < 1) return;
     auto clampi = [](int v, int lo, int hi) { return v < lo ? lo : (v > hi ? hi : v); };
@@ -551,15 +555,19 @@
             const size_t oy = blob.size(); blob.resize(oy + 4 * (size_t)nby);
             memcpy(&blob[oy], ty[i].data(), 32 * (size_t)nby);
             S.tx = reinterpret_cast<const HsPyrStageX*>(ox * 8); S.ty = reinterpret_cast<const HsPyrStageY*>(oy * 8);
+            for (int bx = 0; bx < nbx; bx++) {
+                const size_t oc = hs_pyramid_col_records(xtab[first + i], D.w, txs[i][bx].x0, txs[i][bx].src_x0, cols_blob);
+                if (bx == 0) CC.st[i] = reinterpret_cast<const uint8_t*>(oc);
+            }
         }
         C.tbx = tbx; C.lds_pitch = pitch; C.x_bytes = (int32_t)((x_bytes + 15) & ~(size_t)15); C.h_rows = h_rows; C.grid_x = nbx; C.grid_y = nby; C.valid = 1;
     }
 }
 
 void hs_pyramid_build_tables(const HsLevel* h_lv, int nlevels, const int16_t* const* xtab, const int16_t* const* yofs, const int16_t* const* ibeta,
-                             std::vector<uint64_t>& blob, std::vector<HsPyrFuse>& fuse)
-{
-    fuse.assign(nlevels, HsPyrFuse{});
+                             std::vector<uint64_t>& blob, std::vector<HsPyrFuse>& fuse, std::vector<uint64_t>& cols_blob, std::vector<HsPyrFuseCols>& fuse_cols)
+{
+    fuse.assign(nlevels, HsPyrFuse{}); fuse_cols.assign(nlevels, HsPyrFuseCols{});
     auto clampi = [](int v, int lo, int hi) { return v < lo ? lo : (v > hi ? hi : v); };
     if (blob.empty()) blob.push_back(0);
     for (int l = 1; l + 1 < nlevels; l++) {
@@ -620,6 +628,12 @@
             }
         }
         F.rowA = reinterpret_cast<const HsPyrRow*>(oa * 8); F.rowB = reinterpret_cast<const HsPyrRow*>(ob * 8); F.slotA = slotA;
+        for (int pass = 0; pass < 2; pass++)
+            for (int bx = 0; bx < nbx; bx++) {
+                HsPyrXTile t; memcpy(&t, &blob[ox + 4 * (size_t)bx], 32);
+                const size_t oc = pass == 0 ? hs_pyramid_col_records(xA, A.w, t.ax0, t.col0, cols_blob) : hs_pyramid_col_records(xB, B.w, bx * tbx, t.ax0, cols_blob);
+                if (bx == 0) (pass == 0 ? fuse_cols[l].a : fuse_cols[l].b) = reinterpret_cast<const uint8_t*>(oc);
+            }
     }
 }
 
@@ -672,7 +686,8 @@
     static int v = [] { const char* e = getenv("HS_PYRAMID_NW8"); return e ? atoi(e) : 3; }();
     return v;
 }
-int hs_launch_pyramid(const HsLevel* d_lv, const HsLevel* h_lv, const HsPyrFuse* fuse, const HsPyrChain* chain, int nlevels, HsImg0 img0, int batch, hipStream_t s, const HsPyrChain* deep)
+int hs_launch_pyramid(const HsLevel* d_lv, const HsLevel* h_lv, const HsPyrFuse* fuse, const HsPyrChain* chain, int nlevels, HsImg0 img0, int batch, hipStream_t s, const HsPyrCols& cols,
+                      const HsPyrChain* deep)
 {
     const bool big_lds = deep != nullptr && [] {
         int dev = -1;
@@ -696,8 +711,8 @@
             const size_t lds = (size_t)C.x_bytes + (size_t)C.h_rows * 256 * 2;
             if (vec16 && (lds <= 64 * 1024 || big_lds)) {
                 dim3 grid(C.grid_x, C.grid_y, batch);
-                if ((size_t)grid.x * grid.y * grid.z <= (size_t)256 * pyr_nw8_wg_per_cu()) hipLaunchKernelGGL(k_resize_chain<8>, grid, dim3(512), lds, s, C, img0);
-                else hipLaunchKernelGGL(k_resize_chain<4>, grid, dim3(256), lds, s, C, img0);
+                if ((size_t)grid.x * grid.y * grid.z <= (size_t)256 * pyr_nw8_wg_per_cu()) hipLaunchKernelGGL(k_resize_chain<8>, grid, dim3(512), lds, s, C, img0, cols.deep[l]);
+                else hipLaunchKernelGGL(k_resize_chain<4>, grid, dim3(256), lds, s, C, img0, cols.deep[l]);
                 l += C.nstage - 1;
                 continue;
             }
@@ -709,8 +724,8 @@
                 const HsPyrChain& C = chain[l];
                 const size_t lds = (size_t)C.x_bytes + (size_t)C.h_rows * 256 * 2;
                 dim3 grid(C.grid_x, C.grid_y, batch);
-                if ((size_t)grid.x * grid.y * grid.z <= (size_t)256 * pyr_nw8_wg_per_cu()) hipLaunchKernelGGL(k_resize_chain<8>, grid, dim3(512), lds, s, C, img0);
-                else hipLaunchKernelGGL(k_resize_chain<4>, grid, dim3(256), lds, s, C, img0);
+                if ((size_t)grid.x * grid.y * grid.z <= (size_t)256 * pyr_nw8_wg_per_cu()) hipLaunchKernelGGL(k_resize_chain<8>, grid, dim3(512), lds, s, C, img0, cols.chain[l]);
+                else hipLaunchKernelGGL(k_resize_chain<4>, grid, dim3(256), lds, s, C, img0, cols.chain[l]);
                 l += C.nstage - 1;
                 continue;
             }
@@ -722,8 +737,8 @@
                 const HsLevel& B = h_lv[l + 1];
                 const size_t lds = (size_t)D.fuse_pitch * D.fuse_sr + (size_t)std::max(D.fuse_sr, D.fuse_ar) * 256 * 2;
                 dim3 grid((B.w + D.fuse_tbx - 1) / D.fuse_tbx, (B.h + FZ_ROWS - 1) / FZ_ROWS, batch);
-                if ((size_t)grid.x * grid.y * grid.z <= (size_t)256 * pyr_nw8_wg_per_cu()) hipLaunchKernelGGL(k_resize_two_levels<8>, grid, dim3(512), lds, s, fuse[l], img0);
-                else hipLaunchKernelGGL(k_resize_two_levels<4>, grid, dim3(256), lds, s, fuse[l], img0);
+                if ((size_t)grid.x * grid.y * grid.z <= (size_t)256 * pyr_nw8_wg_per_cu()) hipLaunchKernelGGL(k_resize_two_levels<8>, grid, dim3(512), lds, s, fuse[l], img0, cols.fuse[l]);
+                else hipLaunchKernelGGL(k_resize_two_levels<4>, grid, dim3(256), lds, s, fuse[l], img0, cols.fuse[l]);
                 l++;
                 continue;
             }
@@ -737,7 +752,7 @@
         const size_t lds_bytes = (size_t)lds_pitch * lds_rows + (size_t)lds_rows * 256 * 2;
         if (vec16 && lds_bytes <= 60 * 1024 && scx <= 2.0) {
             dim3 grid((D.w + 255) / 256, (D.h + LT_ROWS - 1) / LT_ROWS, batch);
-            hipLaunchKernelGGL(k_resize_level_lds, grid, dim3(256), lds_bytes, s, d_lv, l, img0, lds_pitch, lds_rows);
+            hipLaunchKernelGGL(k_resize_level_lds, grid, dim3(256), lds_bytes, s, d_lv, l, img0, lds_pitch, lds_rows, cols.level[l]);
             continue;
         }
         dim3 block(64, 4, 1);
```

New measurement: 49110, median of 6. +1.1%, better.
